# Nilau1998/SAC-Agent

Measured on AMD Instinct MI355X. Metric: env-steps/sec (whole node), boat_env exp-6, 65 536 envs/GPU at 1/2/4/8 MI355X, higher is better.
Workload: dtype f64

## Files before the change

sac-agent_amd/csrc/sacenv_boat.hip:

```cpp

#include <hip/hip_runtime.h>
#include <stdint.h>

#include "sacenv.h"
#include "sacenv_boat_arena.h"
#include "sacenv_boat_math.h"
#include "sacenv_boat_wind.h"
#include "sacenv_boat_draw.h"
#include "sacenv_toys.h"
#include "sacenv_boat_owner.h"

#pragma clang fp contract(off)

namespace {


__global__ void k_spline_g(SacenvBoatParams p, double* __restrict__ g) {
  if (threadIdx.x != 0 || blockIdx.x != 0) return;
  const int n = p.n_knots;
  double a[kMaxK][kMaxK], r[kMaxK][kMaxK];
  for (int i = 0; i < n; ++i)
    for (int j = 0; j < n; ++j) a[i][j] = r[i][j] = 0.0;
  a[0][0] = 1.0, a[0][1] = -2.0, a[0][2] = 1.0;
  a[n - 1][n - 3] = 1.0, a[n - 1][n - 2] = -2.0, a[n - 1][n - 1] = 1.0;
  for (int j = 1; j < n - 1; ++j) {
    a[j][j - 1] = 1.0, a[j][j] = 4.0, a[j][j + 1] = 1.0;
    r[j][j - 1] = 1.0, r[j][j] = -2.0, r[j][j + 1] = 1.0;
  }
  for (int c = 0; c < n; ++c) {
    int piv = c;
    for (int i = c + 1; i < n; ++i)
      if (fabs(a[i][c]) > fabs(a[piv][c])) piv = i;
    for (int j = 0; j < n; ++j) {
      double t = a[c][j]; a[c][j] = a[piv][j]; a[piv][j] = t;
      t = r[c][j]; r[c][j] = r[piv][j]; r[piv][j] = t;
    }
    const double d = a[c][c];
    for (int j = 0; j < n; ++j) a[c][j] /= d, r[c][j] /= d;
    for (int i = 0; i < n; ++i) {
      if (i == c) continue;
      const double f = a[i][c];
      if (f == 0.0) continue;
      for (int j = 0; j < n; ++j) a[i][j] -= f * a[c][j], r[i][j] -= f * r[c][j];
    }
  }
  for (int i = 0; i < n; ++i)
    for (int j = 0; j < n; ++j) g[i * n + j] = r[i][j];
}

constexpr int kMaskThreads = 1024;

__global__ void __launch_bounds__(kWave) k_seed(SacenvBoatParams p, Arena A, const uint32_t* __restrict__ seeds) {
  const int e = blockIdx.x * kWave + threadIdx.x;
  if (e < A.nwaves()) A.refill_mask()[e] = 0ull;
  if (e >= p.n_envs) return;
  uint32_t x = seeds[e];
  uint32_t* key = A.mt_key() + (int64_t)e * kMtN;
  for (int i = 0; i < kMtN; ++i) {
    key[i] = x;
    x = 1812433253u * (x ^ (x >> 30)) + (uint32_t)(i + 1);
  }
  A.i32(U_MTPOS)[e] = kMtN;
  A.i32(U_CONS)[e] = 0;
  A.i32(U_FILL)[e] = 0;
}

__global__ void __launch_bounds__(kWave) k_draw(SacenvBoatParams p, Arena A, Tail T, int mode,
                                                const int32_t* __restrict__ ids,
                                                const int32_t* __restrict__ ex_start_y,
                                                const double* __restrict__ ex_knots,
                                                const int32_t* __restrict__ dev_count) {
  __shared__ DrawLds lds;
  const int lane = threadIdx.x;
  const int nq = dev_count != nullptr ? *dev_count : (int)gridDim.x;
  if ((int)blockIdx.x >= nq) return;
  load_g(p, T.g, lds, lane);
  for (int q = blockIdx.x; q < nq; q += gridDim.x) {
    const int e = ids != nullptr ? ids[q] : q;
    if (e < 0 || e >= p.n_envs) continue;
    int32_t start_y;
    int slot = 0;
    if (mode == 2) {
      start_y = draw_episode_wave(p, A, lds, e, 0, lane, ex_start_y + q,
                                  ex_knots != nullptr ? ex_knots + (int64_t)q * 2 * p.n_knots : nullptr);
    } else if (!p.autoreset) {
      start_y = draw_episode_wave(p, A, lds, e, 0, lane, nullptr, nullptr);
    } else if (mode == 0) {
      start_y = draw_episode_wave(p, A, lds, e, 0, lane, nullptr, nullptr);
      if (lane == 0) {
        A.i32(U_CONS)[e] = 0;
        A.i32(U_FILL)[e] = 1;
      }
    } else {
      const int c = A.i32(U_CONS)[e] + 1;
      const int f = A.i32(U_FILL)[e];
      if (c >= f && lane == 0) atomicOr(&A.status()[1], SACENV_STATUS_SLOT_UNDERFLOW);
      slot = c % kSlots;
      start_y = A.i32(U_STARTY)[(int64_t)slot * A.np + e];
      if (lane == 0) A.i32(U_CONS)[e] = c;
      draw_episode_wave(p, A, lds, e, f % kSlots, lane, nullptr, nullptr);
      if (lane == 0) A.i32(U_FILL)[e] = f + 1;
    }
    if (lane == 0) {
      const Obs o = fresh_state(p, A, T, e, start_y, slot);
      store_obs(A.obs() + (int64_t)e * SACENV_OBS_DIM, o);
    }
    __syncthreads();
  }
}

__global__ void __launch_bounds__(1024) k_compact(const uint8_t* __restrict__ done, int n, int aligned,
                                                  int32_t* __restrict__ ids, int32_t* __restrict__ count) {
  __shared__ int wsum[16];
  __shared__ int base_s;
  const int t = threadIdx.x, lane = t & 63, w = t >> 6;
  if (t == 0) base_s = 0;
  __syncthreads();
  for (int64_t c0 = 0; c0 < n; c0 += 1024 * 64) {
    const int64_t e0 = c0 + (int64_t)t * 64;
    uint64_t bits = 0;
    if (aligned && e0 + 64 <= n) {
      const uint4* v = reinterpret_cast<const uint4*>(done + e0);
#pragma unroll
      for (int k = 0; k < 4; ++k) {
        const uint4 x = v[k];
        const uint32_t wds[4] = {x.x, x.y, x.z, x.w};
#pragma unroll
        for (int d = 0; d < 4; ++d)
#pragma unroll
          for (int by = 0; by < 4; ++by)
            if ((wds[d] >> (8 * by)) & 0xffu) bits |= 1ull << (16 * k + 4 * d + by);
      }
    } else {
      for (int j = 0; j < 64 && e0 + j < n; ++j)
        if (done[e0 + j]) bits |= 1ull << j;
    }
    const int cnt = __popcll(bits);
    const int incl = wave_incl_scan(cnt);
    if (lane == 63) wsum[w] = incl;
    __syncthreads();
    int wbase = 0;
    for (int k = 0; k < w; ++k) wbase += wsum[k];
    int pos = base_s + wbase + incl - cnt;
    while (bits) {
      const int j = __ffsll((long long)bits) - 1;
      bits &= bits - 1ull;
      ids[pos++] = (int32_t)(e0 + j);
    }
    __syncthreads();
    if (t == 1023) base_s += wbase + incl;
    __syncthreads();
  }
  if (t == 0) *count = base_s;
}

#ifdef SACENV_STAMPS
#define REFILL_STAMP(slot, ...)                                     \
  do {                                                              \
    asm volatile("" ::__VA_ARGS__);                                 \
    (slot) = __builtin_amdgcn_s_memrealtime();                      \
  } while (0)
constexpr int kRefillStamps = 24;
#else
#define REFILL_STAMP(slot, ...) \
  do {                          \
  } while (0)
#endif

constexpr int kGroupLanes = 16;
constexpr int kGroups = kWave / kGroupLanes;
__global__ void __launch_bounds__(kWave) k_refill(SacenvBoatParams p, Arena A) {
  __shared__ RngLds lds;
  const int lane = threadIdx.x;
#ifdef SACENV_STAMPS
  uint64_t stm[kRefillStamps] = {};
  int n_st = 0;
#endif
  REFILL_STAMP(stm[0], "s"(lane));
  const int total = __builtin_amdgcn_readfirstlane(A.status()[2]);
  REFILL_STAMP(stm[1], "s"(total));
  if (blockIdx.x == 0 && lane == 0) A.status()[0] += 1;
  const int G = (int)gridDim.x;
  const int g = lane / kGroupLanes, gl = lane % kGroupLanes;
  const int nk = p.n_knots;
  const int ndraw = n_curves(p.experiment);
  const int ncurves = owner_curves(p);
  const int need = 2 * nk * ndraw;
  const int nwords = kGroupLanes + need;
  const bool grp_ok = nk <= 8;
  const uint32_t rng = (uint32_t)(2 * p.start_y_half - 1), mask = range_mask32(rng);
  const int np_ = (int)A.np;
  int r0 = blockIdx.x * kGroups;
  int rq = r0 + g < np_ ? r0 + g : 0;
  int e_n = A.refill_list(0)[rq], f_n = A.refill_list(1)[rq], c_n = A.refill_list(2)[rq], p_n = A.cons_snap()[rq];
  for (; r0 < total; r0 += kGroups * G) {
    const int rr = r0 + g;
    const bool ok = rr < total;
    const int e = ok ? e_n : 0;
    const int c = ok ? c_n : 0;
    const int f0 = ok ? f_n : 0;
    const int pos = ok ? (p_n & kMtPosMask) : kMtN;
    const bool nx = ok && (p_n & kMtNextOk) != 0;
    if (r0 + kGroups * G < total) {
      rq = rr + kGroups * G < np_ ? rr + kGroups * G : 0;
      e_n = A.refill_list(0)[rq], f_n = A.refill_list(1)[rq], c_n = A.refill_list(2)[rq], p_n = A.cons_snap()[rq];
    }
    if (ok && c >= f0 && gl == 0) atomicOr(&A.status()[1], SACENV_STATUS_SLOT_UNDERFLOW);
    const int f_end = ok && f0 < c + kSlots ? c + kSlots : f0;
    int f_next = f0, pos_next = pos;
    bool live = ok && f0 < f_end && grp_ok;
    uint32_t* const gw = lds.blk[0] + g * 3 * kGroupLanes;
#pragma unroll 1
    while (__ballot(live) != 0ull) {
      bool fast = live && pos_next + nwords <= (nx ? 2 * kMtN : kMtN);
      const int64_t eo = (int64_t)e * kMtN;
      uint32_t w[3];
#pragma unroll
      for (int q = 0; q < 3; ++q) {
        const int i = pos_next + gl + kGroupLanes * q;
        const uint32_t* src = i < kMtN ? A.mt_key() + eo + i : A.mt_next() + eo + (i - kMtN);
        w[q] = fast && gl + kGroupLanes * q < nwords ? mt_temper(*src) : 0u;
      }
      wave_lds_sync();
#pragma unroll
      for (int q = 0; q < 3; ++q) gw[gl + kGroupLanes * q] = w[q];
      const unsigned long long acc = __ballot(fast && (w[0] & mask) <= rng);
      const uint32_t gacc = (uint32_t)(acc >> (kGroupLanes * g)) & 0xFFFFu;
      fast = fast && gacc != 0u;
      const int k = fast ? __builtin_ctz(gacc) : 0;
      wave_lds_sync();
      REFILL_STAMP(stm[2], "v"(k));
      if (fast) {
        const int slot = f_next % kSlots;
        const int cc = gl / 8, jj = gl % 8;
        if (cc < ncurves && jj < nk) {
          const int src = k + 1 + cc * 2 * nk + 2 * jj;
          const double kv = res53(gw[src], gw[src + 1]);
          A.wind_knots()[2 * A.wix(slot, cc, jj, e)] = kv;
          if (A.rk) A.knots_raw()[A.wix(slot, cc, jj, e)] = kv;
        }
        if (gl == 0) {
          A.i32(U_STARTY)[(int64_t)slot * A.np + e] = -p.start_y_half + (int32_t)(gw[k] & mask);
          A.i32(U_MTPOS)[e] = (pos_next + k + 1 + need) | (nx ? kMtNextOk : 0);
        }
        f_next = f_next + 1;
        pos_next = pos_next + k + 1 + need;
      }
      live = fast && f_next < f_end;
    }
    wave_lds_sync();
#pragma unroll 1
    for (int j = 0; j < kGroups; ++j) {
      const int src = j * kGroupLanes;
      if (__builtin_amdgcn_readlane((int)ok, src) == 0) break;
      const int ej = __builtin_amdgcn_readlane(e, src);
      const int fe = __builtin_amdgcn_readlane(f_end, src);
      int f = __builtin_amdgcn_readlane(f_next, src);
      const int pj = __builtin_amdgcn_readlane(pos_next, src);
      bool first = true;
      for (; f < fe; ++f) {
        const int32_t start_y = draw_knots_wave(p, A, lds, ej, lane, nullptr, nullptr, first ? pj : -1);
#ifdef SACENV_STAMPS
        const int sb = 3 + (n_st < 18 ? n_st : 18);
        ++n_st;
#endif
        REFILL_STAMP(stm[sb], "v"(start_y));
        first = false;
        __syncthreads();
        store_draw(p, A, lds, ej, f % kSlots, start_y, lane, true);
        __syncthreads();
      }
      if (lane == 0) {
        A.i32(U_FILL)[ej] = fe;
        A.refill_list(1)[r0 + j] = __builtin_amdgcn_readlane(f0, src);
        A.refill_list(2)[r0 + j] = fe;
      }
    }
  }
#ifdef SACENV_STAMPS
  stm[22] = __builtin_amdgcn_s_memrealtime();
  stm[23] = (uint64_t)n_st;
  if (lane == 0 && (int64_t)(blockIdx.x + 1) * kRefillStamps * 8 <= 24 * A.np) {
    uint64_t* d = reinterpret_cast<uint64_t*>(A.accel()) + (int64_t)blockIdx.x * kRefillStamps;
    for (int i = 0; i < kRefillStamps; ++i) d[i] = stm[i];
  }
#endif
}

template <int GS, bool kFull>
__global__ void __launch_bounds__(kWave) k_refill_fit(SacenvBoatParams p, Arena A, Tail T) {
  const int lane = threadIdx.x;
  const int ahead = (int)(A.np / kAheadEnvs);
  if ((int)blockIdx.x < ahead) {
    mt_ahead(p, A, (int)blockIdx.x, lane);
    return;
  }
  const int fb = (int)blockIdx.x - ahead, fgrid = (int)gridDim.x - ahead;
  const int nc = p.use_wind_table ? 0 : n_curves(p.experiment);
  const int nk = kFull ? GS : p.n_knots;
  const int items = A.status()[2] * nc;
#ifdef SACENV_STAMPS
  const uint64_t st0 = __builtin_amdgcn_s_memrealtime();
  uint64_t* const fst = reinterpret_cast<uint64_t*>(A.reward64()) + 2 * (int64_t)blockIdx.x;
  const bool fst_ok = lane == 0 && (int64_t)(blockIdx.x + 1) * 16 <= 8 * A.np;
  if (fst_ok) fst[0] = st0, fst[1] = 0;
#endif
  if (items == 0 || fb * (kWave / GS) >= items) return;
  const int j = lane & (GS - 1);
  const int jj = j < nk ? j : nk - 1, j1 = jj + 1 < nk ? jj + 1 : jj;
  double gr[GS];
#pragma unroll
  for (int k = 0; k < GS; ++k) gr[k] = kFull || k < nk ? T.g[jj * nk + k] : 0.0;
  IvGrid ig = interval_grid(p, j < nk - 1 ? j : 0);
  ig.valid = ig.valid && j < nk - 1;
  const int per = kWave / GS;
  for (int base = fb * per; base < items; base += fgrid * per) {
    const int item = base + lane / GS;
    if (item >= items) break;
    fit_group<GS, kFull>(p, A, gr, ig, item, j, jj, j1, nc);
  }
#ifdef SACENV_STAMPS
  __syncthreads();
  if (fst_ok) fst[1] = __builtin_amdgcn_s_memrealtime();
#endif
}

__device__ __forceinline__ unsigned long long lookback_load(const unsigned long long* w) {
  return __hip_atomic_load(w, __ATOMIC_RELAXED, __HIP_MEMORY_SCOPE_AGENT);
}
__global__ void __launch_bounds__(kMaskThreads) k_need_masks(SacenvBoatParams p, Arena A) {
  __shared__ int wcnt[kMaskThreads / kWave];
  const int t = threadIdx.x, lane = t & (kWave - 1), wv = t >> 6;
  const int nw = A.nwaves(), b = (int)blockIdx.x;
  const int w = b * (kMaskThreads / kWave) + wv, e = w * kWave + lane;
  const uint32_t epoch = (uint32_t)A.status()[0] + 1u;
  bool need = false;
  int c = 0, fl = 0, mp = 0;
  if (w < nw && e < p.n_envs) {
    c = A.i32(U_CONS)[e];
    fl = A.i32(U_FILL)[e];
    mp = A.i32(U_MTPOS)[e];
    need = fl < c + kSlots;
  }
  const unsigned long long m = __ballot(need);
  if (lane == 0) wcnt[wv] = __popcll(m);
  __syncthreads();
  if (t < kWave) {
    unsigned long long* const look = A.refill_mask();
    const int cnt = t < kMaskThreads / kWave ? wcnt[t] : 0;
    const int incl = wave_incl_scan(cnt);
    const int total = __builtin_amdgcn_readlane(incl, kMaskThreads / kWave - 1);
    if (t == 0)
      __hip_atomic_store(look + b, ((unsigned long long)epoch << 32) | (uint32_t)total, __ATOMIC_RELAXED,
                         __HIP_MEMORY_SCOPE_AGENT);
    int before = 0;
    for (int q0 = 0; q0 < b; q0 += kWave) {
      const int q = q0 + t;
      unsigned long long x = q < b ? lookback_load(look + q) : ((unsigned long long)epoch << 32);
      for (uint32_t it = 0; __ballot((uint32_t)(x >> 32) != epoch) != 0ull; ++it) {
        if (it >= kSpinLimit) {
          if (t == 0) atomicOr(&A.status()[1], SACENV_STATUS_LIST_TIMEOUT);
          break;
        }
        __builtin_amdgcn_s_sleep(1);
        if ((uint32_t)(x >> 32) != epoch) x = lookback_load(look + q);
      }
      int v = (uint32_t)(x >> 32) == epoch ? (int)(uint32_t)x : 0;
      v += __shfl_xor(v, 32);
      v += __shfl_xor(v, 16);
      v += __shfl_xor(v, 8);
      v += __shfl_xor(v, 4);
      v += __shfl_xor(v, 2);
      v += __shfl_xor(v, 1);
      before += v;
    }
    if (t < kMaskThreads / kWave) wcnt[t] = before + incl - cnt;
    if (t == 0 && b == (int)gridDim.x - 1) A.status()[2] = before + total;
  }
  __syncthreads();
  if (need) {
    const int r = wcnt[wv] + __popcll(m & ((1ull << lane) - 1ull));
    A.refill_list(0)[r] = e;
    A.refill_list(1)[r] = fl;
    A.refill_list(2)[r] = c;
    A.cons_snap()[r] = mp;
  }
}

template <bool kMixed, int kNc, bool kTIdx>
__global__ void __launch_bounds__(kWave) k_step(SacenvBoatParams p, Arena A, Tail T,
                                                const float* __restrict__ action, int nb_boat,
                                                MixedToys M, char* __restrict__ trans) {
  __shared__ OwnerLds slds;
  const int lane = threadIdx.x;
  int b = (int)blockIdx.x;
  if (!kMixed || b < nb_boat) {
    owner_wave<false, kNc, kTIdx>(p, A, T, action, slds, b, lane, 1, nullptr,
                                  trans);
    return;
  }
  b -= nb_boat;
  if (b < M.nb[0]) {
    toy_wave(M.p[0], M.a[0], b, lane);
  } else if (M.n > 1) {
    toy_wave(M.p[1], M.a[1], b - M.nb[0], lane);
  }
}

template <int kNc, bool kTIdx, int kRows, bool kLean = false>
__global__ void __launch_bounds__(kWave) k_rollout(SacenvBoatParams p, Arena A, Tail T,
                                                   const float* __restrict__ action, int n_steps, RollArgs ra) {
  __shared__ OwnerLds slds;
  rollout_body<kNc, kTIdx, kRows, true, kLean>(p, A, T, action, n_steps, ra, slds);
}
template <int kNc, bool kTIdx, int kRows, bool kLean = false>
__global__ void __launch_bounds__(kWave) __attribute__((amdgpu_waves_per_eu(2, 2)))
k_rollout_dense(SacenvBoatParams p, Arena A, Tail T, const float* __restrict__ action, int n_steps, RollArgs ra) {
  __shared__ OwnerLds slds;
  rollout_body<kNc, kTIdx, kRows, false, kLean>(p, A, T, action, n_steps, ra, slds);
}

template <int kNc, bool kTIdx, bool kLean = false>
__global__ void __launch_bounds__(kWave) k_rollout_mixed(SacenvBoatParams p, Arena A, Tail T,
                                                         const float* __restrict__ action, int n_steps, RollArgs ra,
                                                         int nb_boat, MixedToys M) {
  __shared__ OwnerLds slds;
  const int lane = threadIdx.x;
  int b = (int)blockIdx.x;
  if (b < nb_boat) {
    owner_wave<true, kNc, kTIdx, false, 0, true, kLean>(vreg_params(p), A, vreg_tail(T), action, slds, b, lane,
                                                         n_steps, &ra);
    return;
  }
  b -= nb_boat;
  if (b < M.nb[0]) {
    toy_roll_wave(M.p[0], M.a[0], b, lane, n_steps);
  } else if (M.n > 1) {
    toy_roll_wave(M.p[1], M.a[1], b - M.nb[0], lane, n_steps);
  }
}

__global__ void __launch_bounds__(kWave) k_toy_init(SacenvToyParams p, ToyArena T, const int32_t* __restrict__ ids,
                                                    int n, int zero_counters) {
  const int q = blockIdx.x * kWave + threadIdx.x;
  if (q >= n) return;
  const int e = ids != nullptr ? ids[q] : q;
  if (e < 0 || e >= p.n_envs) return;
  double f[5];
  float obs[2];
  toy_initial(p, f, obs);
  for (int k = 0; k < 5; ++k) T.f(k)[e] = f[k];
  T.count()[e] = 0;
  if (zero_counters)
    for (int k = 0; k < 3; ++k) T.ctr(k)[e] = 0u;
  reinterpret_cast<float2*>(T.obs())[e] = make_float2(obs[0], obs[1]);
  T.reward()[e] = 0.0f;
  T.done()[e] = 0;
  T.term()[e] = 0;
}

__global__ void __launch_bounds__(kWave) k_toy_step(SacenvToyParams p, ToyArena T) {
  toy_wave(p, T, blockIdx.x, threadIdx.x);
}

__global__ void __launch_bounds__(256) k_wind_eval(SacenvBoatParams p, Arena A, Tail T,
                                                   const int32_t* __restrict__ env_ids,
                                                   const int32_t* __restrict__ idx, int n,
                                                   double* __restrict__ out_v, double* __restrict__ out_a) {
  const int q = blockIdx.x * blockDim.x + threadIdx.x;
  if (q >= n) return;
  const int e = env_ids[q];
  if (e < 0 || e >= p.n_envs) return;
  const int slot = p.autoreset ? A.i32(U_CONS)[e] % kSlots : 0;
  double wv, wa;
  wind_at(p, A, T.table, slot, e, idx[q], wv, wa);
  out_v[q] = wv;
  out_a[q] = wa;
}


int check_params(const SacenvBoatParams* p) {
  if (p == nullptr) return SACENV_E_NULL;
  if (p->experiment < 1 || p->experiment > 6) return SACENV_E_EXPERIMENT;
  if (p->n_envs <= 0 || p->n_envs > (1 << 22) || p->wind_len <= 0) return SACENV_E_SIZE;
  if (n_curves(p->experiment) > 0 && (p->n_knots < 4 || p->n_knots > kMaxK)) return SACENV_E_KNOTS;
  if (p->n_knots < 2 || p->n_knots > kMaxK) return SACENV_E_KNOTS;
  if (n_curves(p->experiment) > 0 && !p->use_wind_table && p->wind_len < 2) return SACENV_E_SIZE;
  if (p->start_y_half < 1) return SACENV_E_RANGE;
  if (p->autoreset && (p->n_helpers < 1 || p->n_helpers > 65536)) return SACENV_E_SIZE;
  return SACENV_OK;
}

Tail make_tail(const SacenvBoatParams& p, void* arena) {
  const Arena A = make_arena(p, arena);
  Tail T;
  T.g = reinterpret_cast<const double*>(A.b + off_spline_g(A.ur(), A.np));
  T.table = reinterpret_cast<const double*>(A.b + off_wind_table(A.ur(), A.np));
  T.r_mx = 1.0 / p.m_plus_mx;
  T.r_my = 1.0 / p.m_plus_my;
  T.r_iz = 1.0 / p.i_plus_iz;
  T.r_nd = 1.0 / p.n_times_d;
  T.r_w = 1.0 / p.track_width;
  T.r_goal = 1.0 / p.goal_line;
  T.r_two_w = 1.0 / (p.track_width + p.track_width);
  T.r_fuel = 1.0 / (double)p.fuel0;
  T.k_front = p.c_r_front * 0.5 * p.rho * p.boat_area_front;
  T.k_thrust = p.n_squared * p.rho * p.d_pow4 * p.one_minus_td;
  T.k_side = p.c_r_side * 0.5 * p.rho * p.boat_area_side;
  T.k_rud_front = p.c_r_front * 0.5 * p.rho * p.rudder_area;
  T.k_hull = p.c_r_side * 0.5 * p.rho * p.boat_area_side * p.boat_l * 5.0;
  T.k_rud_moment = p.c_r_side * 0.5 * p.rho * p.rudder_area * (p.boat_b / 2);
  return T;
}

int launch_status() {
  const hipError_t err = hipGetLastError();
  return err == hipSuccess ? SACENV_OK : (int)err;
}

inline int blocks_for(int n, int per) { return (n + per - 1) / per; }
inline int owner_waves(const SacenvBoatParams& p) { return (int)(pad64(p.n_envs) / kWave); }

int check_toy(const SacenvToyParams* p) {
  if (p == nullptr) return SACENV_E_NULL;
  if (p->kind != SACENV_TOY_PARACHUTE && p->kind != SACENV_TOY_CAR) return SACENV_E_EXPERIMENT;
  if (p->n_envs <= 0) return SACENV_E_SIZE;
  return SACENV_OK;
}

ToyArena make_toy_arena(const SacenvToyParams& p, void* base) {
  return ToyArena{static_cast<char*>(base), pad64(p.n_envs)};
}

using StepKernel = void (*)(SacenvBoatParams, Arena, Tail, const float*, int, MixedToys, char*);
using RolloutKernel = void (*)(SacenvBoatParams, Arena, Tail, const float*, int, RollArgs);
using MixedRolloutKernel = void (*)(SacenvBoatParams, Arena, Tail, const float*, int, RollArgs, int, MixedToys);
using FitKernel = void (*)(SacenvBoatParams, Arena, Tail);

template <int kNc, bool kTIdx>
struct Owner {
  static constexpr int nc = kNc;
  static constexpr bool ti = kTIdx;
};
template <class F>
auto owner_dispatch(const SacenvBoatParams& p, F f) {
  switch (owner_curves(p) * 2 + (t_from_index(p.dt) ? 1 : 0)) {
    case 0: return f(Owner<0, false>{});
    case 1: return f(Owner<0, true>{});
    case 2: return f(Owner<1, false>{});
    case 3: return f(Owner<1, true>{});
    case 4: return f(Owner<2, false>{});
    default: return f(Owner<2, true>{});
  }
}

StepKernel step_kernel(const SacenvBoatParams& p, bool mixed) {
  return owner_dispatch(p, [mixed](auto o) -> StepKernel {
    using O = decltype(o);
    return mixed ? k_step<true, O::nc, O::ti> : k_step<false, O::nc, O::ti>;
  });
}

bool dense_grid(int nb_boat) {
  int dev = 0, cus = 0;
  if (hipGetDevice(&dev) != hipSuccess ||
      hipDeviceGetAttribute(&cus, hipDeviceAttributeMultiprocessorCount, dev) != hipSuccess)
    return false;
  return nb_boat > 4 * cus;
}

bool lean_launch(const SacenvBoatParams& p, const RollArgs& ra) {
  return p.out_flags == 0 && p.autoreset != 0 && p.experiment != 2 && p.fuel0 != 0 && ra.rec_stride == 0 &&
         ra.fin_stride == 0;
}

int rollout_rows(const RollArgs& ra) {
  return ra.stage != nullptr ? 2 : ra.trans != nullptr ? 1 : ra.rec_stride != 0 ? 3 : 0;
}

template <int kNc, bool kTIdx, int kRows, bool kLean = false>
RolloutKernel rollout_one(bool dense) {
  return dense ? k_rollout_dense<kNc, kTIdx, kRows, kLean> : k_rollout<kNc, kTIdx, kRows, kLean>;
}
RolloutKernel rollout_kernel(const SacenvBoatParams& p, int rows, bool lean, bool dense) {
  return owner_dispatch(p, [=](auto o) -> RolloutKernel {
    constexpr int nc = decltype(o)::nc;
    constexpr bool ti = decltype(o)::ti;
    switch (rows) {
      case 0: return lean ? rollout_one<nc, ti, 0, true>(dense) : rollout_one<nc, ti, 0>(dense);
      case 1: return rollout_one<nc, ti, 1>(dense);
      case 2: return lean ? rollout_one<nc, ti, 2, true>(dense) : rollout_one<nc, ti, 2>(dense);
      default: return rollout_one<nc, ti, 3>(dense);
    }
  });
}

MixedRolloutKernel rollout_mixed_kernel(const SacenvBoatParams& p, bool lean) {
  return owner_dispatch(p, [lean](auto o) -> MixedRolloutKernel {
    using O = decltype(o);
    return lean ? k_rollout_mixed<O::nc, O::ti, true> : k_rollout_mixed<O::nc, O::ti>;
  });
}

FitKernel refill_fit_kernel(int n_knots) {
  return n_knots == 8   ? k_refill_fit<8, true>
         : n_knots < 8  ? k_refill_fit<8, false>
         : n_knots == 16 ? k_refill_fit<16, true>
                         : k_refill_fit<16, false>;
}

RollArgs arena_roll_args(const Arena& A) {
  RollArgs ra{};
  ra.rec = A.b + A.ur() * A.np;
  ra.fin = reinterpret_cast<float*>(ra.rec + R_FIN * A.np);
  ra.status = reinterpret_cast<int32_t*>(A.b + off_status(A.ur(), A.np)) + 1;
  return ra;
}

int launch_multi(const SacenvBoatParams& p, void* arena, const float* actions, int n_steps, const RollArgs& ra,
                 void* stream) {
  const int nb_boat = owner_waves(p);
  const RolloutKernel k = rollout_kernel(p, rollout_rows(ra), lean_launch(p, ra), dense_grid(nb_boat));
  hipLaunchKernelGGL(k, dim3(nb_boat), dim3(kWave), 0, (hipStream_t)stream, p, make_arena(p, arena),
                     make_tail(p, arena), actions, n_steps, ra);
  return launch_status();
}

struct MixedLaunch {
  MixedToys M{};
  SacenvBoatParams p{};
  Arena A{};
  Tail T{};
  int nb_boat = 0, nb = 0;
};
int mixed_setup(const SacenvBoatParams* bp, void* boat_arena, const float* boat_actions,
                const SacenvToyParams* toy_params, void* const* toy_arenas, int32_t n_toys, int32_t n_steps,
                MixedLaunch* L) {
  int rc;
  if (n_toys < 0 || n_toys > 2) return SACENV_E_SIZE;
  if (n_toys > 0 && (toy_params == nullptr || toy_arenas == nullptr)) return SACENV_E_NULL;
  if (n_steps < 1) return SACENV_E_SIZE;
  L->M.n = n_toys;
  for (int t = 0; t < n_toys; ++t) {
    if ((rc = check_toy(&toy_params[t]))) return rc;
    if (toy_arenas[t] == nullptr) return SACENV_E_NULL;
    L->M.p[t] = toy_params[t];
    L->M.a[t] = make_toy_arena(toy_params[t], toy_arenas[t]);
    L->M.nb[t] = blocks_for(toy_params[t].n_envs, kWave);
    L->nb += L->M.nb[t];
  }
  if (bp != nullptr) {
    if ((rc = check_params(bp))) return rc;
    if (boat_arena == nullptr || boat_actions == nullptr) return SACENV_E_NULL;
    L->p = *bp;
    L->A = make_arena(*bp, boat_arena);
    L->T = make_tail(*bp, boat_arena);
    L->nb_boat = owner_waves(*bp);
    L->nb += L->nb_boat;
  }
  return SACENV_OK;
}

}

extern "C" {

int sacenv_abi_version(void) { return SACENV_ABI_VERSION; }

int sacenv_stream_create_exclusive(void** stream) {
  if (stream == nullptr) return SACENV_E_NULL;
  int dev = 0;
  hipError_t e = hipGetDevice(&dev);
  if (e != hipSuccess) return (int)e;
  hipDeviceProp_t prop;
  e = hipGetDeviceProperties(&prop, dev);
  if (e != hipSuccess) return (int)e;
  uint32_t mask[64];
  const int words = (prop.multiProcessorCount + 31) / 32;
  if (words > 64) return SACENV_E_SIZE;
  for (int i = 0; i < words; ++i) mask[i] = 0xFFFFFFFFu;
  hipStream_t s = nullptr;
  e = hipExtStreamCreateWithCUMask(&s, (uint32_t)words, mask);
  if (e != hipSuccess) return (int)e;
  *stream = s;
  return SACENV_OK;
}

int sacenv_stream_destroy(void* stream) {
  if (stream == nullptr) return SACENV_E_NULL;
  return (int)hipStreamDestroy((hipStream_t)stream);
}

const char* sacenv_error_string(int code) {
  switch (code) {
    case SACENV_OK: return "ok";
    case SACENV_E_NULL: return "required pointer is NULL";
    case SACENV_E_EXPERIMENT: return "Well someone tried to use an experiment that doesnt exist!";
    case SACENV_E_KNOTS:
      return "Please select at least 4 fixed_points in your config. The interpolation doesn't work "
             "otherwise! (max 16)";
    case SACENV_E_SIZE: return "size out of range";
    case SACENV_E_RANGE: return "low >= high: int(0.8*track_width) must be >= 1";
    case SACENV_E_MODE: return "call not valid in this autoreset mode";
    default: return code > 0 ? hipGetErrorString((hipError_t)code) : "unknown sacenv error";
  }
}

int sacenv_boat_layout(const SacenvBoatParams* p, SacenvBoatLayout* out) {
  const int rc = check_params(p);
  if (rc) return rc;
  if (out == nullptr) return SACENV_E_NULL;
  compute_layout(p->n_envs, p->n_knots, p->wind_len, p->use_wind_table, (p->out_flags & SACENV_OUT_KNOTS) != 0, out);
  return SACENV_OK;
}

int sacenv_boat_init(const SacenvBoatParams* p, void* arena, const uint32_t* seeds, void* stream) {
  int rc = check_params(p);
  if (rc) return rc;
  if (arena == nullptr || seeds == nullptr) return SACENV_E_NULL;
  const hipStream_t s = (hipStream_t)stream;
  const Arena A = make_arena(*p, arena);
  const Tail T = make_tail(*p, arena);
  hipLaunchKernelGGL(k_spline_g, dim3(1), dim3(1), 0, s, *p, const_cast<double*>(T.g));
  if ((rc = launch_status())) return rc;
  hipLaunchKernelGGL(k_seed, dim3(blocks_for(p->n_envs, kWave)), dim3(kWave), 0, s, *p, A, seeds);
  if ((rc = launch_status())) return rc;
  hipLaunchKernelGGL(k_draw, dim3(p->n_envs), dim3(kWave), 0, s, *p, A, T, 0, (const int32_t*)nullptr,
                     (const int32_t*)nullptr, (const double*)nullptr, (const int32_t*)nullptr);
  if ((rc = launch_status())) return rc;
  return p->autoreset ? sacenv_boat_refill(p, arena, stream) : SACENV_OK;
}

int sacenv_boat_reset(const SacenvBoatParams* p, void* arena, const int32_t* ids, int32_t n_ids,
                      void* stream) {
  int rc = check_params(p);
  if (rc) return rc;
  if (arena == nullptr) return SACENV_E_NULL;
  const int nb = ids != nullptr ? n_ids : p->n_envs;
  if (nb < 0) return SACENV_E_SIZE;
  if (nb == 0) return SACENV_OK;
  const hipStream_t s = (hipStream_t)stream;
  const Arena A = make_arena(*p, arena);
  const Tail T = make_tail(*p, arena);
  hipLaunchKernelGGL(k_draw, dim3(nb), dim3(kWave), 0, s, *p, A, T, 1, ids, (const int32_t*)nullptr,
                     (const double*)nullptr, (const int32_t*)nullptr);
  return launch_status();
}

int sacenv_compact_done(const uint8_t* done, int32_t n, int32_t* ids, int32_t* count, void* stream) {
  if (n < 0) return SACENV_E_SIZE;
  if (count == nullptr || (n > 0 && (done == nullptr || ids == nullptr))) return SACENV_E_NULL;
  const int aligned = (reinterpret_cast<uintptr_t>(done) & 15u) == 0;
  hipLaunchKernelGGL(k_compact, dim3(1), dim3(1024), 0, (hipStream_t)stream, done, n, aligned, ids, count);
  return launch_status();
}

int sacenv_boat_reset_list(const SacenvBoatParams* p, void* arena, const int32_t* ids, const int32_t* count,
                           void* stream) {
  int rc = check_params(p);
  if (rc) return rc;
  if (arena == nullptr || ids == nullptr || count == nullptr) return SACENV_E_NULL;
  const hipStream_t s = (hipStream_t)stream;
  const Arena A = make_arena(*p, arena);
  const Tail T = make_tail(*p, arena);
  const int grid = p->n_envs < 1024 ? p->n_envs : 1024;
  hipLaunchKernelGGL(k_draw, dim3(grid), dim3(kWave), 0, s, *p, A, T, 1, ids, (const int32_t*)nullptr,
                     (const double*)nullptr, count);
  return launch_status();
}

int sacenv_boat_reset_explicit(const SacenvBoatParams* p, void* arena, const int32_t* ids, int32_t n_ids,
                               const int32_t* start_y, const double* knots, void* stream) {
  int rc = check_params(p);
  if (rc) return rc;
  if (p->autoreset) return SACENV_E_MODE;
  if (arena == nullptr || ids == nullptr || start_y == nullptr) return SACENV_E_NULL;
  if (n_curves(p->experiment) > 0 && !p->use_wind_table && knots == nullptr) return SACENV_E_NULL;
  if (n_ids < 0) return SACENV_E_SIZE;
  if (n_ids == 0) return SACENV_OK;
  hipLaunchKernelGGL(k_draw, dim3(n_ids), dim3(kWave), 0, (hipStream_t)stream, *p, make_arena(*p, arena),
                     make_tail(*p, arena), 2, ids, start_y, knots, (const int32_t*)nullptr);
  return launch_status();
}

static int boat_step(const SacenvBoatParams* p, void* arena, const float* action, char* trans, void* stream) {
  int rc = check_params(p);
  if (rc) return rc;
  if (arena == nullptr || action == nullptr) return SACENV_E_NULL;
  const int nb_boat = owner_waves(*p);
  hipLaunchKernelGGL(step_kernel(*p, false), dim3(nb_boat), dim3(kWave), 0, (hipStream_t)stream, *p,
                     make_arena(*p, arena), make_tail(*p, arena), action, nb_boat, MixedToys{}, trans);
  return launch_status();
}

int sacenv_boat_step(const SacenvBoatParams* p, void* arena, const float* action, void* stream) {
  return boat_step(p, arena, action, nullptr, stream);
}

int sacenv_boat_step_pooled(const SacenvBoatParams* p, void* arena, const float* action, void* trans,
                            void* stream) {
  if (trans == nullptr) return SACENV_E_NULL;
  if ((reinterpret_cast<uintptr_t>(trans) & 15u) != 0u) return SACENV_E_RANGE;
  return boat_step(p, arena, action, static_cast<char*>(trans), stream);
}

int sacenv_boat_rollout(const SacenvBoatParams* p, void* arena, const float* actions, int32_t n_steps,
                        void* records, float* final_obs, void* stream) {
  int rc = check_params(p);
  if (rc) return rc;
  if (arena == nullptr || actions == nullptr || records == nullptr) return SACENV_E_NULL;
  if (n_steps < 1 || (p->autoreset && n_steps > SACENV_REFILL_PERIOD)) return SACENV_E_SIZE;
  const int64_t np = pad64(p->n_envs);
  RollArgs ra{};
  ra.rec = static_cast<char*>(records);
  ra.rec_stride = SACENV_RECORD_BYTES * np;
  ra.fin = final_obs;
  ra.fin_stride = np * SACENV_OBS_DIM;
  ra.act_stride = p->n_envs;
  return launch_multi(*p, arena, actions, n_steps, ra, stream);
}

int sacenv_boat_segment(const SacenvBoatParams* p, void* arena, const float* actions, int64_t action_stride,
                        int32_t n_steps, const uint32_t* act_ready, uint32_t* step_done, uint32_t seq0,
                        void* trans, int64_t trans_stride, void* stage, uint64_t* stage_marks,
                        void* stream) {
  int rc = check_params(p);
  if (rc) return rc;
  if (arena == nullptr || actions == nullptr) return SACENV_E_NULL;
  if (n_steps < 1 || (p->autoreset && n_steps > SACENV_REFILL_PERIOD)) return SACENV_E_SIZE;
  if (action_stride < p->n_envs ||
      ((act_ready != nullptr || step_done != nullptr) && (uint64_t)seq0 + (uint64_t)n_steps >= 0x80000000ull))
    return SACENV_E_RANGE;
  if (trans != nullptr && ((reinterpret_cast<uintptr_t>(trans) & 15u) != 0u || (trans_stride & 15) != 0))
    return SACENV_E_RANGE;
  if (stage != nullptr && (trans != nullptr || (reinterpret_cast<uintptr_t>(stage) & 15u) != 0u))
    return SACENV_E_RANGE;
  if (stage_marks != nullptr && n_steps > SACENV_REFILL_PERIOD) return SACENV_E_SIZE;
  RollArgs ra = arena_roll_args(make_arena(*p, arena));
  ra.trans = static_cast<char*>(trans);
  ra.trans_stride = trans_stride;
  ra.stage = static_cast<char*>(stage);
  ra.marks = reinterpret_cast<unsigned long long*>(stage_marks);
  ra.act_stride = action_stride;
  ra.ready = act_ready;
  ra.done = step_done;
  ra.seq0 = seq0;
  return launch_multi(*p, arena, actions, n_steps, ra, stream);
}

int sacenv_boat_segment_occupancy(const SacenvBoatParams* p, int32_t with_trans, int32_t* blocks_per_cu,
                                  int32_t* grid, int32_t* vgprs, int32_t* lds_bytes) {
  int rc = check_params(p);
  if (rc) return rc;
  if (blocks_per_cu == nullptr || grid == nullptr || vgprs == nullptr || lds_bytes == nullptr) return SACENV_E_NULL;
  const int nb_boat = owner_waves(*p);
  const int rows = with_trans == 2 ? 2 : with_trans ? 1 : 0;
  const RolloutKernel k = rollout_kernel(*p, rows, lean_launch(*p, RollArgs{}), dense_grid(nb_boat));
  int nb = 0;
  hipFuncAttributes fa{};
  hipError_t e = hipOccupancyMaxActiveBlocksPerMultiprocessor(&nb, k, kWave, 0);
  if (e == hipSuccess) e = hipFuncGetAttributes(&fa, reinterpret_cast<const void*>(k));
  if (e != hipSuccess) return (int)e;
  *blocks_per_cu = nb;
  *grid = nb_boat;
  *vgprs = fa.numRegs;
  *lds_bytes = (int32_t)fa.sharedSizeBytes;
  return SACENV_OK;
}

int sacenv_boat_refill(const SacenvBoatParams* p, void* arena, void* stream) {
  int rc = check_params(p);
  if (rc) return rc;
  if (arena == nullptr) return SACENV_E_NULL;
  if (!p->autoreset) return SACENV_E_MODE;
  const Arena A = make_arena(*p, arena);
  const unsigned mask_blocks = (unsigned)((A.np / kWave + kMaskThreads / kWave - 1) / (kMaskThreads / kWave));
  hipLaunchKernelGGL(k_need_masks, dim3(mask_blocks), dim3(kMaskThreads), 0, (hipStream_t)stream, *p, A);
  if ((rc = launch_status())) return rc;
  hipLaunchKernelGGL(k_refill, dim3(p->n_helpers), dim3(kWave), 0, (hipStream_t)stream, *p, A);
  if ((rc = launch_status())) return rc;
  const int fit_blocks = 8192 + (int)(A.np / kAheadEnvs);
  hipLaunchKernelGGL(refill_fit_kernel(p->n_knots), dim3(fit_blocks), dim3(kWave), 0, (hipStream_t)stream, *p, A,
                     make_tail(*p, arena));
  return launch_status();
}

int sacenv_toy_layout(const SacenvToyParams* p, SacenvToyLayout* out) {
  const int rc = check_toy(p);
  if (rc) return rc;
  if (out == nullptr) return SACENV_E_NULL;
  toy_layout(p->n_envs, out);
  return SACENV_OK;
}

int sacenv_toy_init(const SacenvToyParams* p, void* arena, void* stream) {
  const int rc = check_toy(p);
  if (rc) return rc;
  if (arena == nullptr) return SACENV_E_NULL;
  hipLaunchKernelGGL(k_toy_init, dim3(blocks_for(p->n_envs, kWave)), dim3(kWave), 0, (hipStream_t)stream, *p,
                     make_toy_arena(*p, arena), (const int32_t*)nullptr, p->n_envs, 1);
  return launch_status();
}

int sacenv_toy_reset(const SacenvToyParams* p, void* arena, const int32_t* ids, int32_t n_ids, void* stream) {
  const int rc = check_toy(p);
  if (rc) return rc;
  if (arena == nullptr) return SACENV_E_NULL;
  const int n = ids != nullptr ? n_ids : p->n_envs;
  if (n < 0) return SACENV_E_SIZE;
  if (n == 0) return SACENV_OK;
  hipLaunchKernelGGL(k_toy_init, dim3(blocks_for(n, kWave)), dim3(kWave), 0, (hipStream_t)stream, *p,
                     make_toy_arena(*p, arena), ids, n, 0);
  return launch_status();
}

int sacenv_toy_step(const SacenvToyParams* p, void* arena, void* stream) {
  const int rc = check_toy(p);
  if (rc) return rc;
  if (arena == nullptr) return SACENV_E_NULL;
  hipLaunchKernelGGL(k_toy_step, dim3(blocks_for(p->n_envs, kWave)), dim3(kWave), 0, (hipStream_t)stream, *p,
                     make_toy_arena(*p, arena));
  return launch_status();
}

static int mixed_step(const SacenvBoatParams* bp, void* boat_arena, const float* boat_action,
                      const SacenvToyParams* toy_params, void* const* toy_arenas, int32_t n_toys,
                      char* trans, void* stream) {
  MixedLaunch L;
  const int rc = mixed_setup(bp, boat_arena, boat_action, toy_params, toy_arenas, n_toys, 1, &L);
  if (rc) return rc;
  if (L.nb == 0) return SACENV_OK;
  hipLaunchKernelGGL(step_kernel(L.p, true), dim3(L.nb), dim3(kWave), 0, (hipStream_t)stream, L.p, L.A, L.T,
                     boat_action, L.nb_boat, L.M, trans);
  return launch_status();
}

int sacenv_mixed_step(const SacenvBoatParams* bp, void* boat_arena, const float* boat_action,
                      const SacenvToyParams* toy_params, void* const* toy_arenas, int32_t n_toys,
                      void* stream) {
  return mixed_step(bp, boat_arena, boat_action, toy_params, toy_arenas, n_toys, nullptr, stream);
}

int sacenv_mixed_step_pooled(const SacenvBoatParams* bp, void* boat_arena, const float* boat_action,
                             const SacenvToyParams* toy_params, void* const* toy_arenas, int32_t n_toys,
                             void* trans, void* stream) {
  if (bp == nullptr || trans == nullptr) return SACENV_E_NULL;
  if ((reinterpret_cast<uintptr_t>(trans) & 15u) != 0u) return SACENV_E_RANGE;
  return mixed_step(bp, boat_arena, boat_action, toy_params, toy_arenas, n_toys, static_cast<char*>(trans),
                    stream);
}

int sacenv_mixed_segment(const SacenvBoatParams* bp, void* boat_arena, const float* boat_actions,
                         int64_t action_stride, int32_t n_steps, const SacenvToyParams* toy_params,
                         void* const* toy_arenas, int32_t n_toys, void* stream) {
  MixedLaunch L;
  const int rc = mixed_setup(bp, boat_arena, boat_actions, toy_params, toy_arenas, n_toys, n_steps, &L);
  if (rc) return rc;
  RollArgs ra{};
  if (bp != nullptr) {
    if (bp->autoreset && n_steps > SACENV_REFILL_PERIOD) return SACENV_E_SIZE;
    if (action_stride < bp->n_envs) return SACENV_E_RANGE;
    ra = arena_roll_args(L.A);
    ra.act_stride = action_stride;
  }
  if (L.nb == 0) return SACENV_OK;
  hipLaunchKernelGGL(rollout_mixed_kernel(L.p, lean_launch(L.p, ra)), dim3(L.nb), dim3(kWave), 0,
                     (hipStream_t)stream, L.p, L.A, L.T, boat_actions, n_steps, ra, L.nb_boat, L.M);
  return launch_status();
}

int sacenv_boat_wind_eval(const SacenvBoatParams* p, const void* arena, const int32_t* env_ids,
                          const int32_t* idx, int32_t n, double* out_velocity, double* out_angle,
                          void* stream) {
  int rc = check_params(p);
  if (rc) return rc;
  if (!arena || !env_ids || !idx || !out_velocity || !out_angle) return SACENV_E_NULL;
  if (n < 0) return SACENV_E_SIZE;
  if (n == 0) return SACENV_OK;
  void* a = const_cast<void*>(arena);
  hipLaunchKernelGGL(k_wind_eval, dim3(blocks_for(n, 256)), dim3(256), 0, (hipStream_t)stream, *p,
                     make_arena(*p, a), make_tail(*p, a), env_ids, idx, n, out_velocity, out_angle);
  return launch_status();
}

}
```

sac-agent_amd/csrc/sacenv_boat_arena.h:

```cpp
#pragma once

#include <hip/hip_runtime.h>
#include <stdint.h>
#include <string.h>

#include "sacenv.h"

namespace {
constexpr int kWave = 64;
}

#include "mt19937.h"

namespace {

constexpr int kMaxK = SACENV_MAX_KNOTS;
constexpr int kSlots = SACENV_SLOTS;
constexpr double kPi = 3.141592653589793;

constexpr int U_SX = 0, U_SY = 8, U_SR = 16, U_VX = 24, U_VY = 32, U_VR = 40, U_RUD = 48,
              U_EP = 56, U_COEF = 64, U_W0N = 128, U_T = 144, U_IDX = 152,
              U_CONS = 156, U_FILL = 160, U_MTPOS = 164, U_SYN = 168, U_STARTY = 172,
              U_CNT = U_STARTY + 4 * kSlots,
              U_LIST = U_CNT + 4 * SACENV_N_COUNTERS, U_CSNAP = U_LIST + 12, U_LTERM = U_CSNAP + 4,
              U_WIND = U_LTERM + 4;
constexpr int U_MT_BYTES = 4 * kMtN;
constexpr int kMtPosMask = 0xFFFF, kMtNextOk = 1 << 16;
constexpr int U_PAIRED = 144;
constexpr int64_t kWindUnits = 16LL * kSlots;

__host__ __device__ inline int64_t pad64(int64_t n) { return (n + 63) / 64 * 64; }
__host__ __device__ inline int64_t align256(int64_t x) { return (x + 255) / 256 * 256; }

constexpr int R_OBS = SACENV_REC_OBS, R_REWARD = SACENV_REC_REWARD, R_DONE = SACENV_REC_DONE,
              R_TERM = SACENV_REC_TERM, R_FIN = SACENV_RECORD_BYTES,
              R_FIN_EP = R_FIN + 4 * SACENV_OBS_DIM,
              R_AX = R_FIN_EP + 8, R_AY = R_AX + 8, R_AR = R_AY + 8,
              R_REWARD64 = R_AR + 8, R_END = R_REWARD64 + 8;
static_assert(R_OBS == 0 && R_REWARD == 4 * SACENV_OBS_DIM && R_DONE == R_REWARD + 4 && R_TERM == R_DONE + 1 &&
                  SACENV_RECORD_BYTES == R_TERM + 1,
              "record: obs f32 x 11, reward f32, done u8, term u8");
static_assert(R_FIN == 50 && R_FIN_EP == 94 && R_AX == 102 && R_AY == 110 && R_AR == 118 && R_REWARD64 == 126 &&
                  R_END == 134,
              "the arena columns behind the record (SacenvBoatLayout, ABI 20)");
static_assert(R_FIN_EP % 2 == 0 && (R_AX - R_FIN_EP) % 8 == 0, "f64 columns stay 8-B aligned (n_pad % 64 == 0)");

__host__ __device__ inline int64_t record_unit(int nk, int rk) {
  return U_WIND + (2 + rk) * (kWindUnits * nk) + 2 * U_MT_BYTES;
}
__host__ __device__ inline int64_t off_refill_mask(int64_t ur, int64_t np) { return align256((ur + R_END) * np); }
__host__ __device__ inline int64_t refill_mask_bytes(int64_t np) { return align256(8 * (int)(np / 64)); }
__host__ __device__ inline int64_t off_status(int64_t ur, int64_t np) {
  return off_refill_mask(ur, np) + refill_mask_bytes(np);
}
__host__ __device__ inline int64_t off_spline_g(int64_t ur, int64_t np) { return off_status(ur, np) + 256; }
__host__ __device__ inline int64_t off_wind_table(int64_t ur, int64_t np) {
  return off_spline_g(ur, np) + align256(8LL * kMaxK * kMaxK);
}

__host__ __device__ inline void compute_layout(int n, int nk, int L, int use_table, int raw_knots,
                                               SacenvBoatLayout* o) {
  const int64_t np = pad64(n);
  o->n_pad = np;
  auto pair_off = [np](int u) { return (int64_t)(u & ~15) * np + (u & 8); };
  o->s_x = pair_off(U_SX);
  o->s_y = pair_off(U_SY);
  o->s_r = pair_off(U_SR);
  o->v_x = pair_off(U_VX);
  o->v_y = pair_off(U_VY);
  o->v_r = pair_off(U_VR);
  o->rudder = pair_off(U_RUD);
  o->t = U_T * np;
  o->ep_reward = pair_off(U_EP);
  o->wind_coef = U_COEF * np;
  o->wind0_next = U_W0N * np;
  o->start_y_next = U_SYN * np;
  o->index = U_IDX * np;
  o->cons = U_CONS * np;
  o->fill = U_FILL * np;
  o->mt_pos = U_MTPOS * np;
  o->start_y = U_STARTY * np;
  o->counters = U_CNT * np;
  o->refill_list = U_LIST * np;
  const int64_t uw = U_WIND, wk = kWindUnits * nk, rk = raw_knots ? 1 : 0;
  o->wind_knots = uw * np;
  o->knots_raw = raw_knots ? (uw + 2 * wk) * np : -1;
  o->mt_key = (uw + (2 + rk) * wk) * np;
  o->mt_next = o->mt_key + U_MT_BYTES * np;
  const int64_t ur = record_unit(nk, (int)rk);
  o->record = ur * np;
  o->obs = (ur + R_OBS) * np;
  o->reward = (ur + R_REWARD) * np;
  o->done = (ur + R_DONE) * np;
  o->term = (ur + R_TERM) * np;
  o->final_obs = (ur + R_FIN) * np;
  o->final_ep_reward = (ur + R_FIN_EP) * np;
  o->accel = (ur + R_AX) * np;
  o->reward64 = (ur + R_REWARD64) * np;
  o->refill_mask = off_refill_mask(ur, np);
  o->status = off_status(ur, np);
  o->spline_g = off_spline_g(ur, np);
  o->wind_table = off_wind_table(ur, np);
  o->total_bytes = o->wind_table + (use_table ? align256(16LL * L) : 0);
  o->last_term = U_LTERM * np;
}

struct Arena {
  char* b;
  int64_t np;
  int nk;
  int rk;
  template <class T>
  __device__ __forceinline__ T* at(int64_t units) const { return reinterpret_cast<T*>(b + units * np); }
  __device__ __forceinline__ int32_t* i32(int u) const { return at<int32_t>(u); }
  __device__ __forceinline__ int nwaves() const { return (int)(np / 64); }
  __device__ __forceinline__ int64_t wk() const { return kWindUnits * nk; }
  __device__ __forceinline__ double* wind_knots() const { return at<double>(U_WIND); }
  __device__ __forceinline__ double* knots_raw() const { return at<double>(U_WIND + 2 * wk()); }
  __device__ __forceinline__ uint32_t* mt_key() const { return at<uint32_t>(U_WIND + (2 + rk) * wk()); }
  __device__ __forceinline__ uint32_t* mt_next() const { return mt_key() + kMtN * np; }
  __host__ __device__ __forceinline__ int64_t ur() const { return record_unit(nk, rk); }
  __device__ __forceinline__ float* obs() const { return at<float>(ur() + R_OBS); }
  __device__ __forceinline__ float* final_obs() const { return at<float>(ur() + R_FIN); }
  __device__ __forceinline__ double* accel() const { return at<double>(ur() + R_AX); }
  __device__ __forceinline__ double* reward64() const { return at<double>(ur() + R_REWARD64); }
  __device__ __forceinline__ char* tail() const { return b + off_refill_mask(ur(), np); }
  __device__ __forceinline__ unsigned long long* refill_mask() const {
    return reinterpret_cast<unsigned long long*>(tail());
  }

  __device__ __forceinline__ int32_t* cons_snap() const { return i32(U_CSNAP); }
  __device__ __forceinline__ int32_t* status() const {
    return reinterpret_cast<int32_t*>(tail() + refill_mask_bytes(np));
  }
  __device__ __forceinline__ int32_t* refill_list(int k) const { return i32(U_LIST + 4 * k); }
  __device__ __forceinline__ int64_t wix(int slot, int c, int k, int e) const {
    return (((int64_t)e * kSlots + slot) * 2 + c) * nk + k;
  }
  __device__ __forceinline__ const char* wk_wave(int e0) const {
    return reinterpret_cast<const char*>(wind_knots()) + (int64_t)e0 * (int64_t)kSlots * 32 * nk;
  }
  __device__ __forceinline__ uint32_t wko_l(int slot, int c, int k, int l) const {
    return ((((uint32_t)l * (uint32_t)kSlots + (uint32_t)slot) * 2u + (uint32_t)c) * (uint32_t)nk + (uint32_t)k) * 16u;
  }
  __device__ __forceinline__ void piece_at(const char* wbase, uint32_t off, double (&q)[4]) const {
    const char* base = wbase + off;
    const double2 a = *reinterpret_cast<const double2*>(base), b = *reinterpret_cast<const double2*>(base + 16);
    q[0] = a.x, q[1] = a.y, q[2] = b.x, q[3] = b.y;
  }
  __device__ __forceinline__ void piece(int slot, int c, int k, int e, double (&q)[4]) const {
    piece_at(wk_wave(e & ~63), wko_l(slot, c, k, e & 63), q);
  }
  template <class T>
  __device__ __forceinline__ T& at_e(int64_t unit, uint32_t off) const {
    return *reinterpret_cast<T*>(b + unit * np + off);
  }
  template <class T>
  __device__ __forceinline__ T& at_s(int u, uint32_t off) const {
    return *reinterpret_cast<T*>(b + ((uint32_t)u * (uint32_t)np + off));
  }
  __device__ __forceinline__ double& f64e(int u, uint32_t eo) const {
    return u < U_PAIRED ? at_s<double>(u & ~15, 2u * eo + (uint32_t)(u & 8)) : at_s<double>(u, eo);
  }
  __device__ __forceinline__ double2& f64p(int u, uint32_t eo) const { return at_s<double2>(u, 2u * eo); }
  __device__ __forceinline__ int32_t& i32e(int u, uint32_t eo4) const { return at_s<int32_t>(u, eo4); }
};

__host__ inline Arena make_arena(const SacenvBoatParams& p, void* base) {
  return Arena{static_cast<char*>(base), pad64(p.n_envs), p.n_knots, (p.out_flags & SACENV_OUT_KNOTS) ? 1 : 0};
}

struct Tail {
  const double* g;
  const double* table;
  double r_mx, r_my, r_iz, r_nd, r_w;
  double r_goal, r_two_w, r_fuel;
  double k_front, k_thrust, k_side, k_rud_front, k_hull, k_rud_moment;
};

__host__ __device__ __forceinline__ int n_curves(int experiment) {
  return experiment == 6 ? 2 : (experiment == 4 || experiment == 5) ? 1 : 0;
}
__host__ __device__ __forceinline__ int owner_curves(const SacenvBoatParams& p) {
  return p.use_wind_table ? 0 : n_curves(p.experiment);
}

__host__ __device__ inline bool t_from_index(double dt) {
  uint64_t bits;
  memcpy(&bits, &dt, sizeof bits);
  return (bits & ((1ull << 30) - 1ull)) == 0ull;
}

}
```

sac-agent_amd/csrc/sacenv_boat_draw.h:

```cpp
#pragma once

#include <hip/hip_runtime.h>
#include <stdint.h>

#include "sacenv.h"
#include "sacenv_boat_arena.h"
#include "sacenv_boat_math.h"
#include "sacenv_boat_wind.h"
#include "mt19937.h"

#pragma clang fp contract(off)

namespace {

struct RngLds {
  uint32_t win[kWave];
  uint32_t blk[2][kMtN];
  double y[2][kMaxK];
};
struct DrawLds : RngLds {
  double m[2][kMaxK];
  double g[kMaxK * kMaxK];
};


__device__ __forceinline__ void load_g(const SacenvBoatParams& p, const double* g, DrawLds& l, int lane) {
  for (int i = lane; i < p.n_knots * p.n_knots; i += kWave) l.g[i] = g[i];
  __syncthreads();
}


__device__ int32_t draw_knots_wave(const SacenvBoatParams& p, const Arena& A, RngLds& l, int e,
                                   int lane, const int32_t* ex_start_y, const double* ex_knots,
                                   int pos0 = -1, bool have_w0 = false, uint32_t w0_pre = 0u) {
  const int nk = p.n_knots;
  const int ndraw = n_curves(p.experiment);
  const int ncurves = owner_curves(p);
  if (ex_start_y != nullptr) {
    for (int c = 0; c < ncurves; ++c)
      if (lane < nk) l.y[c][lane] = ex_knots[c * nk + lane];
    return *ex_start_y;
  }
  MtStream st;
  st.gkey = A.mt_key() + (int64_t)e * kMtN;
  st.pos = pos0 >= 0 ? pos0 : A.i32(U_MTPOS)[e] & kMtPosMask;
  st.cur = 0;
  st.loaded = false;
  st.nxt_valid = false;
  st.advanced = false;
  const uint32_t rng = (uint32_t)(2 * p.start_y_half - 1), mask = range_mask32(rng);
  uint32_t val = 0;
  const int need = 2 * nk * ndraw;
  const uint32_t w0 = have_w0 ? mt_temper(w0_pre) : mt_fetch(st, l, lane);
  const unsigned long long acc0 = __ballot(((w0 & mask) <= rng) && lane < kWave - need);
  if (acc0) {
    const int k = __ffsll((long long)acc0) - 1;
    val = (uint32_t)__builtin_amdgcn_readlane((int)w0, k) & mask;
    if (ndraw > 0) {
      l.win[lane] = w0;
      __syncthreads();
    }
    for (int c = 0; c < ndraw; ++c) {
      const int src = k + 1 + c * 2 * nk + ((2 * lane) & 31);
      const uint32_t wa = l.win[src & (kWave - 1)];
      const uint32_t wb = l.win[(src + 1) & (kWave - 1)];
      if (lane < nk) l.y[c][lane] = res53(wa, wb);
    }
    st.pos += k + 1 + need;
  } else {
    for (;;) {
      const uint32_t w = mt_fetch(st, l, lane);
      const unsigned long long acc = __ballot((w & mask) <= rng);
      if (acc) {
        const int k = __ffsll((long long)acc) - 1;
        val = (uint32_t)__builtin_amdgcn_readlane((int)w, k) & mask;
        st.pos += k + 1;
        break;
      }
      st.pos += kWave;
    }
    for (int c = 0; c < ndraw; ++c) {
      const uint32_t w = mt_fetch(st, l, lane);
      l.win[lane] = w;
      __syncthreads();
      const uint32_t wa = l.win[(2 * lane) & (kWave - 1)];
      const uint32_t wb = l.win[(2 * lane + 1) & (kWave - 1)];
      if (lane < nk) l.y[c][lane] = res53(wa, wb);
      __syncthreads();
      st.pos += 2 * nk;
    }
  }
  mt_finish(st, l, A.i32(U_MTPOS) + e, lane);
  return -p.start_y_half + (int32_t)val;
}

__device__ void fit_store_wave(const SacenvBoatParams& p, const Arena& A, DrawLds& l, int e, int slot,
                               int lane) {
  const int nk = p.n_knots;
  const int ncurves = owner_curves(p);
  if (ncurves == 0) return;
  __syncthreads();
  const int c = lane >> 4, j = lane & 15;
  const bool knot_lane = c < ncurves && j < nk;
  double yv = 0.0, mv = 0.0;
  if (knot_lane) {
    yv = l.y[c][j];
#pragma unroll
    for (int k = 0; k < kMaxK; ++k)
      if (k < nk) mv += l.g[j * nk + k] * l.y[c][k];
    l.m[c][j] = mv;
  }
  __syncthreads();
  double mn = INFINITY, mx = -INFINITY;
  {
    const int cc = lane >> 5, u = lane & 31;
    if (nk - 1 <= 8) {
      const int jj = u >> 2;
      if (cc < ncurves && jj < nk - 1)
        interval_extrema<4>(p, jj, u & 3, l.y[cc][jj], l.y[cc][jj + 1], l.m[cc][jj], l.m[cc][jj + 1], mn, mx);
    } else {
      if (cc < ncurves && u < nk - 1)
        interval_extrema<1>(p, u, 0, l.y[cc][u], l.y[cc][u + 1], l.m[cc][u], l.m[cc][u + 1], mn, mx);
    }
  }
  mn = group_min<16>(mn);
  mx = group_max<16>(mx);
  const double cmn0 = fmin(readlane_f64(mn, 0), readlane_f64(mn, 16));
  const double cmx0 = fmax(readlane_f64(mx, 0), readlane_f64(mx, 16));
  const double cmn1 = fmin(readlane_f64(mn, 32), readlane_f64(mn, 48));
  const double cmx1 = fmax(readlane_f64(mx, 32), readlane_f64(mx, 48));
  mn = c == 0 ? cmn0 : cmn1;
  mx = c == 0 ? cmx0 : cmx1;
  if (knot_lane) {
    fold_knot(p, c, mn, mx, yv, mv);
    *reinterpret_cast<double2*>(A.wind_knots() + 2 * A.wix(slot, c, j, e)) = double2{yv, mv};
  }
  __syncthreads();
}

__device__ __forceinline__ void store_draw(const SacenvBoatParams& p, const Arena& A, const RngLds& l,
                                           int e, int slot, int32_t start_y, int lane, bool raw = false) {
  const int nk = p.n_knots;
  const int ncurves = owner_curves(p);
  if (lane == 0) A.i32(U_STARTY)[(int64_t)slot * A.np + e] = start_y;
  const int c = lane >> 4, j = lane & 15;
  if (c < ncurves && j < nk) {
    if (raw) A.wind_knots()[2 * A.wix(slot, c, j, e)] = l.y[c][j];
    if (A.rk) A.knots_raw()[A.wix(slot, c, j, e)] = l.y[c][j];
  }
}

__device__ int32_t draw_episode_wave(const SacenvBoatParams& p, const Arena& A, DrawLds& l, int e,
                                     int slot, int lane, const int32_t* ex_start_y,
                                     const double* ex_knots) {
  const int32_t start_y = draw_knots_wave(p, A, l, e, lane, ex_start_y, ex_knots);
  __syncthreads();
  store_draw(p, A, l, e, slot, start_y, lane);
  fit_store_wave(p, A, l, e, slot, lane);
  return start_y;
}

__device__ __forceinline__ Obs fresh_state(const SacenvBoatParams& p, const Arena& A, const Tail& T, int e,
                                           int32_t start_y, int slot) {
  const double s_y = p.experiment == 2 ? (double)start_y : 0.0;
  const int nc = owner_curves(p);
  const uint32_t eo = (uint32_t)e * 8u;
  for (int c = 0; c < nc; ++c) {
    double q[4];
    A.piece(slot, c, 0, e, q);
    for (int k = 0; k < 4; ++k) A.f64e(U_COEF + 32 * c + 8 * k, eo) = q[k];
  }
  A.f64e(U_SX, eo) = 0.0;
  A.f64e(U_SY, eo) = s_y;
  A.f64e(U_SR, eo) = 0.0;
  A.f64e(U_VX, eo) = 0.0;
  A.f64e(U_VY, eo) = 0.0;
  A.f64e(U_VR, eo) = 0.0;
  A.f64e(U_RUD, eo) = 0.0;
  A.f64e(U_T, eo) = 0.0;
  A.f64e(U_EP, eo) = 0.0;
  A.i32(U_IDX)[e] = 0;
  if (p.out_flags & SACENV_OUT_ACCEL) {
    A.at_e<double>(A.ur() + R_AX, eo) = 0.0;
    A.at_e<double>(A.ur() + R_AY, eo) = 0.0;
    A.at_e<double>(A.ur() + R_AR, eo) = 0.0;
  }
  return make_obs(p, obs_const(T), 0.0, 0.0, 0.0, s_y, 0.0, 0.0, 0.0, 0.0, 0.0, 0.0, (double)p.fuel0);
}

constexpr int kAheadEnvs = 8;
__device__ __forceinline__ void mt_twist_regs(const uint32_t* o, uint32_t* n, uint32_t* cur, int lane) {
  constexpr int kD = kMtN - kMtM;
  uint32_t a0[4], a1[4], a2[4], b0[4], b1[4], c0[4], c1[4];
#pragma unroll
  for (int k = 0; k < 4; ++k) {
    const int c = lane + kWave * k;
    const bool ok = c < kD, okc = c < kMtN - 1 - 2 * kD;
    a0[k] = ok ? o[c] : 0u;
    a1[k] = ok ? o[c + 1] : 0u;
    a2[k] = ok ? o[c + kMtM] : 0u;
    b0[k] = ok ? o[c + kD] : 0u;
    b1[k] = ok ? o[c + kD + 1] : 0u;
    c0[k] = okc ? o[c + 2 * kD] : 0u;
    c1[k] = okc ? o[c + 2 * kD + 1] : 0u;
  }
  const uint32_t last = o[kMtN - 1];
  asm volatile("s_waitcnt vmcnt(0)" ::: "memory");
  uint32_t nb2 = 0u, na0 = 0u;
#pragma unroll
  for (int k = 0; k < 4; ++k) {
    const int c = lane + kWave * k;
    if (c < kD) {
      const uint32_t na = mt_mix(a0[k], a1[k], a2[k]);
      const uint32_t nb = mt_mix(b0[k], b1[k], na);
      n[c] = na;
      n[c + kD] = nb;
      if (cur) cur[c] = a0[k], cur[c + kD] = b0[k];
      if (c < kMtN - 1 - 2 * kD) {
        n[c + 2 * kD] = mt_mix(c0[k], c1[k], nb);
        if (cur) cur[c + 2 * kD] = c0[k];
      }
      if (k == 0) na0 = na;
      if (k == 2) nb2 = nb;
    }
  }
  const uint32_t n0 = (uint32_t)__builtin_amdgcn_readlane((int)na0, 0);
  const uint32_t n396 = (uint32_t)__builtin_amdgcn_readlane((int)nb2, kMtM - 1 - kD - 2 * kWave);
  if (lane == 0) {
    n[kMtN - 1] = mt_mix(last, n0, n396);
    if (cur) cur[kMtN - 1] = last;
  }
}

__device__ __forceinline__ void mt_ahead(const SacenvBoatParams& p, const Arena& A, int b, int lane) {
  const int e0 = b * kAheadEnvs;
  int v = 0;
  bool need = false;
  if (lane < kAheadEnvs && e0 + lane < p.n_envs && p.n_knots <= 8) {
    v = A.i32(U_MTPOS)[e0 + lane];
    need = (v & kMtNextOk) == 0 || (v & kMtPosMask) > kMtN;
  }
  unsigned long long m = __ballot(need);
#pragma unroll 1
  while (m != 0ull) {
    const int j = __ffsll((long long)m) - 1;
    m &= m - 1ull;
    const int e = e0 + j;
    const int vj = __builtin_amdgcn_readlane(v, j);
    const bool adv = (vj & kMtNextOk) != 0 && (vj & kMtPosMask) > kMtN;
    uint32_t* const key = A.mt_key() + (int64_t)e * kMtN;
    uint32_t* const nxt = A.mt_next() + (int64_t)e * kMtN;
    mt_twist_regs(adv ? nxt : key, nxt, adv ? key : nullptr, lane);
    if (lane == 0) A.i32(U_MTPOS)[e] = ((vj & kMtPosMask) - (adv ? kMtN : 0)) | kMtNextOk;
  }
}

}
```

sac-agent_amd/csrc/sacenv_boat_wind.h:

```cpp
#pragma once

#include <hip/hip_runtime.h>
#include <stdint.h>

#include "sacenv.h"
#include "sacenv_boat_arena.h"

#pragma clang fp contract(off)

namespace {

struct Knot {
  int j;
  double t;
};

__device__ __forceinline__ Knot knot_coord(const SacenvBoatParams& p, int i) {
  const double s = (double)i * p.knot_step;
  int j = (int)s;
  if (j > p.n_knots - 2) j = p.n_knots - 2;
  return Knot{j, s - (double)j};
}

__device__ __forceinline__ double spline_piece(double y0, double y1, double m0, double m1, double t) {
  const double u = 1.0 - t;
  return u * y0 + t * y1 + (u * u * u - u) * m0 + (t * t * t - t) * m1;
}

__device__ __forceinline__ double curve_env(const SacenvBoatParams& p, const Arena& A, int slot, int c,
                                            int e, int i) {
  const Knot k = knot_coord(p, i);
  double q[4];
  A.piece(slot, c, k.j, e, q);
  return spline_piece(q[0], q[2], q[1], q[3], k.t);
}

__device__ __forceinline__ void wind_at(const SacenvBoatParams& p, const Arena& A, const double* table,
                                        int slot, int e, int idx, double& wv, double& wa) {
  if (idx > p.wind_len - 1) idx = p.wind_len - 1;
  if (idx < 0) idx = 0;
  if (p.use_wind_table) {
    wv = table[idx];
    wa = table[p.wind_len + idx];
    return;
  }
  switch (p.experiment) {
    case 3:
      wv = p.max_velocity;
      wa = p.wind_dir_rad;
      return;
    case 4:
      wv = curve_env(p, A, slot, 0, e, idx);
      wa = p.wind_dir_rad;
      return;
    case 5: {
      wv = p.max_velocity;
      const double r = curve_env(p, A, slot, 0, e, idx) <= 0.5 / 2 ? 0.0 : 1.0;
      wa = (r * kPi) + kPi / 2;
      return;
    }
    case 6:
      wv = curve_env(p, A, slot, 0, e, idx);
      wa = curve_env(p, A, slot, 1, e, idx);
      return;
    default:
      wv = 0.0;
      wa = 0.0;
      return;
  }
}


template <int kCtrl>
__device__ __forceinline__ double dpp_f64(double v) {
  const int lo = __builtin_amdgcn_mov_dpp(__double2loint(v), kCtrl, 0xF, 0xF, false);
  const int hi = __builtin_amdgcn_mov_dpp(__double2hiint(v), kCtrl, 0xF, 0xF, false);
  return __hiloint2double(hi, lo);
}
template <int GS>
__device__ __forceinline__ double group_min(double v) {
  v = fmin(v, dpp_f64<0xB1>(v));
  v = fmin(v, dpp_f64<0x4E>(v));
  v = fmin(v, dpp_f64<0x141>(v));
  if (GS == 16) v = fmin(v, dpp_f64<0x140>(v));
  return v;
}
template <int GS>
__device__ __forceinline__ double group_max(double v) {
  v = fmax(v, dpp_f64<0xB1>(v));
  v = fmax(v, dpp_f64<0x4E>(v));
  v = fmax(v, dpp_f64<0x141>(v));
  if (GS == 16) v = fmax(v, dpp_f64<0x140>(v));
  return v;
}
__device__ __forceinline__ double next_lane_f64(double v) {
  const int lo = __builtin_amdgcn_update_dpp(__double2loint(v), __double2loint(v), 0x101, 0xF, 0xF, false);
  const int hi = __builtin_amdgcn_update_dpp(__double2hiint(v), __double2hiint(v), 0x101, 0xF, 0xF, false);
  return __hiloint2double(hi, lo);
}
__device__ __forceinline__ double readlane_f64(double v, int src) {
  return __hiloint2double(__builtin_amdgcn_readlane(__double2hiint(v), src),
                          __builtin_amdgcn_readlane(__double2loint(v), src));
}
__device__ __forceinline__ void wave_lds_sync() {
  __builtin_amdgcn_fence(__ATOMIC_RELEASE, "wavefront");
  __builtin_amdgcn_wave_barrier();
  __builtin_amdgcn_fence(__ATOMIC_ACQUIRE, "wavefront");
}
__device__ __forceinline__ int wave_incl_scan(int x) {
  x += __builtin_amdgcn_update_dpp(0, x, 0x111, 0xF, 0xF, true);
  x += __builtin_amdgcn_update_dpp(0, x, 0x112, 0xF, 0xF, true);
  x += __builtin_amdgcn_update_dpp(0, x, 0x114, 0xF, 0xF, true);
  x += __builtin_amdgcn_update_dpp(0, x, 0x118, 0xF, 0xF, true);
  x += __builtin_amdgcn_update_dpp(0, x, 0x142, 0xA, 0xF, false);
  x += __builtin_amdgcn_update_dpp(0, x, 0x143, 0xC, 0xF, false);
  return x;
}


struct IvGrid {
  double jd, lod, hid;
  bool valid;
};
__device__ __forceinline__ IvGrid interval_grid(const SacenvBoatParams& p, int j) {
  const int L = p.wind_len;
  int lo = (int)ceil((double)j * p.knot_inv) - 1;
  if (lo < 0) lo = 0;
  while (lo < L && knot_coord(p, lo).j < j) ++lo;
  int hi = (int)floor((double)(j + 1) * p.knot_inv) + 1;
  if (hi > L - 1) hi = L - 1;
  while (hi >= 0 && knot_coord(p, hi).j > j) --hi;
  return IvGrid{(double)j, (double)lo, (double)hi, lo <= hi};
}

template <int S>
__device__ __forceinline__ void interval_extrema_on(const SacenvBoatParams& p, const IvGrid& gr, int s,
                                                    double y0, double y1, double a, double b, double& mn,
                                                    double& mx) {
  mn = INFINITY;
  mx = -INFINITY;
  if (!gr.valid) return;
  const double inv = p.knot_inv;
  const double qa = 3.0 * (b - a), qb = 6.0 * a, qc = y1 - y0 - 2.0 * a - b;
  const double c1 = qc, c2 = 3.0 * a, c3 = b - a;
  double r0 = -1.0, r1 = -1.0;
  const double scale = fabs(qa) + fabs(qb) + fabs(qc);
  if (fabs(qa) <= 1e-14 * scale) {
    if (qb != 0.0) r0 = -qc * __builtin_amdgcn_rcp(qb);
  } else {
    double sa = qa, sb = qb, sc = qc;
    if (scale < 0x1p-500) {
      const int up = -__builtin_amdgcn_frexp_exp(scale);
      sa = ldexp(qa, up), sb = ldexp(qb, up), sc = ldexp(qc, up);
    }
    const double disc = sb * sb - 4.0 * sa * sc;
    if (disc >= 0.0) {
      const double sq = disc > 0.0 ? disc * __builtin_amdgcn_rsq(disc) : 0.0;
      const double q = -0.5 * (sb + copysign(sq, sb));
      r0 = q * __builtin_amdgcn_rcp(sa);
      if (q != 0.0) r1 = sc * __builtin_amdgcn_rcp(q);
    }
  }
  const bool ok0 = r0 > -0.01 && r0 < 1.01, ok1 = r1 > -0.01 && r1 < 1.01;
  const double jd = gr.jd, lod = gr.lod, hid = gr.hid;
  const double i0 = ok0 ? floor((jd + r0) * inv) : lod;
  const double i1 = ok1 ? floor((jd + r1) * inv) : lod;
#pragma unroll
  for (int t = 0; t < (10 + S - 1) / S; ++t) {
    const int q = s + S * t;
    double i;
    if (q == 0) {
      i = lod;
    } else if (q == 1) {
      i = hid;
    } else {
      const bool first = q < 6;
      const double d = (double)((first ? q - 2 : q - 6) - 1);
      const bool ok = first ? ok0 : ok1;
      i = fmin(fmax((first ? i0 : i1) + d, lod), hid);
      i = ok ? i : lod;
    }
    if (q < 10) {
      const double t = i * p.knot_step - jd;
      const double v = fma(fma(fma(c3, t, c2), t, c1), t, y0);
      mn = fmin(mn, v);
      mx = fmax(mx, v);
    }
  }
}
template <int S>
__device__ __forceinline__ void interval_extrema(const SacenvBoatParams& p, int j, int s, double y0,
                                                 double y1, double a, double b, double& mn,
                                                 double& mx) {
  interval_extrema_on<S>(p, interval_grid(p, j), s, y0, y1, a, b, mn, mx);
}

__device__ __forceinline__ void fold_knot(const SacenvBoatParams& p, int c, double mn, double mx, double& yv,
                                          double& mv) {
  if (mn < 0.0 || mx > 1.0) {
    const double span = mx - mn;
    yv = (yv - mn) / span;
    mv = mv / span;
  }
  if (p.experiment == 4 || (p.experiment == 6 && c == 0)) {
    yv = yv * p.max_velocity;
    mv = mv * p.max_velocity;
  } else if (p.experiment == 6 && c == 1) {
    yv = yv * kPi * 2;
    mv = mv * kPi * 2;
  }
}

template <int GS, bool kFull>
__device__ __forceinline__ void fit_group(const SacenvBoatParams& p, const Arena& A, const double (&gr)[GS],
                                          const IvGrid& ig, int item, int j, int jj, int j1, int nc) {
  const int nk = kFull ? GS : p.n_knots;
  const int rr = item / nc, c = item - rr * nc;
  const int e = A.refill_list(0)[rr], f0 = A.refill_list(1)[rr], f1 = A.refill_list(2)[rr];
  for (int f = f0; f < f1; ++f) {
    const int slot = f % kSlots;
    const double* kr = A.wind_knots() + 2 * A.wix(slot, c, 0, e);
    double yk[GS];
#pragma unroll
    for (int k = 0; k < GS; ++k) yk[k] = kr[2 * (kFull || k < nk ? k : nk - 1)];
    double yv = kr[2 * jj];
    const double y1 = kr[2 * j1];
    double mv = 0.0;
#pragma unroll
    for (int k = 0; k < GS; ++k) {
      const double s = mv + gr[k] * yk[k];
      mv = kFull || k < nk ? s : mv;
    }
    const double m1 = next_lane_f64(mv);
    double mn, mx;
    interval_extrema_on<1>(p, ig, 0, yv, y1, mv, m1, mn, mx);
    mn = group_min<GS>(mn);
    mx = group_max<GS>(mx);
    if (kFull || j < nk) {
      fold_knot(p, c, mn, mx, yv, mv);
      *reinterpret_cast<double2*>(A.wind_knots() + 2 * A.wix(slot, c, j, e)) = double2{yv, mv};
    }
  }
}

}
```

sac-agent_amd/sacenv/vec_env.py:

```python
from __future__ import annotations

import ctypes as C

import numpy as np
import torch

from . import _lib
from .config import BoatConfig, make_params, observation_bounds, t_from_index
from .spaces import Box

RECORD_BYTES = _lib.RECORD_BYTES


class VecBoatEnv:

    def __init__(self, config=None, num_envs: int = 1, *, seed: int = 0, seeds=None,
                 device=None, max_episode_steps: int = 0, autoreset: bool = True,
                 env_id_offset: int = 0, record_knots: bool = False, record_accel: bool = False,
                 record_reward64: bool = False, wind_table=None, n_helpers: int | None = None,
                 auto_refill: bool = True):
        self.lib = _lib.load()
        self.cfg = BoatConfig.from_any(config)
        self.num_envs = N = int(num_envs)
        if N <= 0:
            raise ValueError("num_envs must be positive")
        self.device = _lib.cuda_device(device, "VecBoatEnv")
        self.env_id_offset = int(env_id_offset)
        self.autoreset = bool(autoreset)
        self.auto_refill = bool(auto_refill)
        self._since_refill = 0
        if n_helpers is None:
            n_helpers = max(1024, ((N + 63) // 64 * 64) * 3 // 16)
        flags = ((_lib.OUT_KNOTS if record_knots else 0) | (_lib.OUT_ACCEL if record_accel else 0)
                 | (_lib.OUT_REWARD64 if record_reward64 else 0))
        self.params = make_params(self.cfg, N, max_episode_steps=max_episode_steps,
                                  autoreset=autoreset, n_helpers=n_helpers, out_flags=flags,
                                  use_wind_table=wind_table is not None)
        self._pp = C.byref(self.params)
        self.layout = L = _lib.layout(self.params)
        self.n_pad = NP = int(L.n_pad)
        self.arena = torch.zeros(int(L.total_bytes), dtype=torch.uint8, device=self.device)
        nk = int(self.cfg.fixed_points)

        def view(off, dtype, *shape):
            esz = torch.empty((), dtype=dtype).element_size()
            cnt = int(np.prod(shape))
            return self.arena[off: off + cnt * esz].view(dtype).view(*shape)

        f64, i32 = torch.float64, torch.int32

        def pair_view(off):
            k = (off % 16) // 8
            return view(off - 8 * k, f64, NP, 2)[:N, k]

        for name in ("s_x", "s_y", "s_r", "v_x", "v_y", "v_r", "rudder", "ep_reward"):
            setattr(self, name, pair_view(getattr(L, name)))
        self._t_view = view(L.t, f64, NP)[:N]
        self._t_from_index = t_from_index(float(self.cfg.dt))
        self.index = view(L.index, i32, NP)[:N]
        self.cons = view(L.cons, i32, NP)[:N]
        self.mt_pos = view(L.mt_pos, i32, NP)[:N]
        self.start_y_slots = view(L.start_y, i32, _lib.SLOTS, NP)[:, :N]
        self.counters = view(L.counters, i32, _lib.N_COUNTERS, NP)[:, :N]
        self.last_term = view(L.last_term, i32, NP)[:N]
        self.wind_knots = view(L.wind_knots, f64, NP, _lib.SLOTS, 2, nk, 2)
        self.knots_raw_slots = view(L.knots_raw, f64, NP, _lib.SLOTS, 2, nk) if record_knots else None
        self.mt_key = view(L.mt_key, i32, NP, _lib.MT_N)[:N]
        self.mt_next = view(L.mt_next, i32, NP, _lib.MT_N)[:N]
        self.spline_g = view(L.spline_g, f64, nk, nk)
        self.record = self.arena[L.record: L.record + RECORD_BYTES * NP]
        self.obs = view(L.obs, torch.float32, NP, _lib.OBS_DIM)[:N]
        self.reward = view(L.reward, torch.float32, NP)[:N]
        self.done = view(L.done, torch.uint8, NP)[:N]
        self.term = view(L.term, torch.uint8, NP)[:N]
        self.final_obs = view(L.final_obs, torch.float32, NP, _lib.OBS_DIM)[:N]
        self.final_obs_bytes = self.arena[L.final_obs: L.final_obs + 4 * _lib.OBS_DIM * NP]
        self.final_ep_reward = view(L.final_ep_reward, f64, NP)[:N]
        self.accel = view(L.accel, f64, 3, NP)[:, :N]
        self.reward64 = view(L.reward64, f64, NP)[:N]
        self.status = view(L.status, i32, 64)
        if wind_table is not None:
            wt = torch.as_tensor(np.asarray(wind_table, np.float64).reshape(2, -1))
            if wt.shape[1] != self.cfg.wind_len:
                raise ValueError("wind_table must be [2, int(t_max/dt)]")
            view(L.wind_table, f64, 2, self.cfg.wind_len).copy_(wt)

        self.action_space = Box(low=-1, high=1, dtype=np.float32)
        low, high = observation_bounds()
        self.observation_space = Box(low=low, high=high, dtype=np.float32)

        if seeds is None:
            gid = np.arange(N, dtype=np.uint64) + np.uint64(self.env_id_offset)
            seeds = (np.uint64(seed) + gid) & np.uint64(0xFFFFFFFF)
        seeds = np.asarray(seeds, dtype=np.uint64)
        if seeds.shape != (N,):
            raise ValueError("seeds must have one entry per env")
        if np.any(seeds > 0xFFFFFFFF):
            raise ValueError("Seed must be between 0 and 2**32 - 1")
        self.seeds = seeds
        self._seeds_dev = torch.from_numpy(seeds.astype(np.uint32).view(np.int32)).to(self.device)
        _lib.check(self.lib.sacenv_boat_init(self._pp, self._ptr, self._seeds_dev.data_ptr(),
                                             self.stream))

    @property
    def mt_index(self) -> torch.Tensor:
        return self.mt_pos & 0xFFFF

    @property
    def _ptr(self) -> int:
        return self.arena.data_ptr()

    @property
    def stream(self) -> int:
        return torch.cuda.current_stream(self.device).cuda_stream

    @property
    def t(self) -> torch.Tensor:
        if self._t_from_index:
            return self.index.to(torch.float64) * float(self.cfg.dt)
        return self._t_view

    @property
    def start_y(self) -> torch.Tensor:
        slot = (self.cons % _lib.SLOTS).long() if self.autoreset else torch.zeros_like(self.cons).long()
        return self.start_y_slots.gather(0, slot[None, :])[0]

    @property
    def knots_raw(self) -> torch.Tensor:
        if self.knots_raw_slots is None:
            raise RuntimeError("construct the env with record_knots=True to keep the drawn knots")
        slot = (self.cons % _lib.SLOTS).long() if self.autoreset else torch.zeros_like(self.cons).long()
        k = self.knots_raw_slots[: self.num_envs]
        return k[torch.arange(self.num_envs, device=k.device), slot].permute(1, 2, 0)

    def reset(self, env_ids=None) -> torch.Tensor:
        if env_ids is None:
            _lib.check(self.lib.sacenv_boat_reset(self._pp, self._ptr, None, 0, self.stream))
        else:
            ids = torch.as_tensor(env_ids, dtype=torch.int32, device=self.device).contiguous()
            if ids.numel():
                _lib.check(self.lib.sacenv_boat_reset(self._pp, self._ptr, ids.data_ptr(),
                                                      ids.numel(), self.stream))
                self._keep = ids
        return self.obs

    def compact_done(self, done=None):
        d = self.done if done is None else torch.as_tensor(done, dtype=torch.uint8, device=self.device)
        d = d.contiguous()
        ids = torch.empty(d.numel(), dtype=torch.int32, device=self.device)
        count = torch.empty(1, dtype=torch.int32, device=self.device)
        _lib.check(self.lib.sacenv_compact_done(d.data_ptr(), d.numel(), ids.data_ptr(),
                                                count.data_ptr(), self.stream))
        self._keep_c = d
        return ids, count

    def reset_done(self, done=None) -> torch.Tensor:
        ids, count = self.compact_done(done)
        _lib.check(self.lib.sacenv_boat_reset_list(self._pp, self._ptr, ids.data_ptr(),
                                                   count.data_ptr(), self.stream))
        self._keep = (ids, count)
        return self.obs

    def reset_explicit(self, env_ids, start_y, knots=None) -> torch.Tensor:
        ids = torch.as_tensor(env_ids, dtype=torch.int32, device=self.device).contiguous()
        sy = torch.as_tensor(start_y, dtype=torch.int32, device=self.device).contiguous()
        kn = None
        if knots is not None:
            kn = torch.as_tensor(knots, dtype=torch.float64, device=self.device).contiguous()
        _lib.check(self.lib.sacenv_boat_reset_explicit(
            self._pp, self._ptr, ids.data_ptr(), ids.numel(), sy.data_ptr(),
            None if kn is None else kn.data_ptr(), self.stream))
        self._keep = (ids, sy, kn)
        return self.obs

    def check_actions(self, actions: torch.Tensor) -> None:
        if not isinstance(actions, torch.Tensor):
            raise TypeError("actions must be a torch tensor on the env's device")
        if actions.dtype != torch.float32 or not actions.is_contiguous():
            raise ValueError("actions must be a contiguous float32 tensor")
        if actions.numel() != self.num_envs:
            raise ValueError(f"actions must hold num_envs={self.num_envs} values, got {actions.numel()}")
        if actions.device != self.device:
            raise ValueError(f"actions are on {actions.device}, the env on {self.device}")

    def step_async(self, actions: torch.Tensor) -> None:
        self.check_actions(actions)
        _lib.check(self.lib.sacenv_boat_step(self._pp, self._ptr, actions.data_ptr(), self.stream))
        self._after_step()

    def step_pooled_async(self, actions: torch.Tensor, trans_row: torch.Tensor) -> None:
        self.check_actions(actions)
        nb = _lib.trans_bytes(self.params.experiment) * self.n_pad
        if (trans_row.dtype != torch.uint8 or trans_row.device != self.device
                or trans_row.numel() != nb or not trans_row.is_contiguous()):
            raise ValueError(f"trans_row must be a contiguous uint8 device tensor of {nb} bytes")
        _lib.check(self.lib.sacenv_boat_step_pooled(self._pp, self._ptr, actions.data_ptr(),
                                                    trans_row.data_ptr(), self.stream))
        self._after_step()

    def first_obs_template(self) -> torch.Tensor:
        from .config import first_obs_template
        return torch.from_numpy(first_obs_template(self.cfg))

    def rollout(self, actions, records=None, final_obs=None):
        a = torch.as_tensor(actions, device=self.device)
        if a.dtype != torch.float32:
            a = a.to(torch.float32)
        K = int(a.shape[0])
        a = a.reshape(K, self.num_envs).contiguous()
        if self.autoreset and K > _lib.REFILL_PERIOD:
            raise ValueError(f"rollout of more than {_lib.REFILL_PERIOD} steps in autoreset mode")
        if self.autoreset and self.auto_refill and self._since_refill + K > _lib.REFILL_PERIOD:
            self.refill()
        if records is None:
            records = torch.empty((K, RECORD_BYTES * self.n_pad), dtype=torch.uint8, device=self.device)
        _lib.check(self.lib.sacenv_boat_rollout(
            self._pp, self._ptr, a.data_ptr(), K, records.data_ptr(),
            None if final_obs is None else final_obs.data_ptr(), self.stream))
        self._keep_roll = a
        if self.autoreset:
            self._since_refill += K
        return records, final_obs

    def segment_async(self, actions: torch.Tensor, n_steps: int | None = None, *, act_ready=None,
                      step_done=None, seq0: int = 0, trans=None, trans_stride: int = 0, stage=None,
                      stage_marks=None) -> None:
        K = int(actions.shape[0]) if n_steps is None else int(n_steps)
        if (not isinstance(actions, torch.Tensor) or actions.dtype != torch.float32
                or actions.device != self.device or actions.dim() != 2
                or actions.shape[1] != self.num_envs or actions.stride(1) != 1 or actions.shape[0] < K):
            raise ValueError(f"actions must be a float32 [>= {K}, {self.num_envs}] device tensor with "
                             "contiguous rows")
        if self.autoreset and K > _lib.REFILL_PERIOD:
            raise ValueError(f"a segment of more than {_lib.REFILL_PERIOD} steps in autoreset mode")
        if self.autoreset and self.auto_refill and self._since_refill + K > _lib.REFILL_PERIOD:
            self.refill()
        nw = self.n_pad // 64
        for name, f in (("act_ready", act_ready), ("step_done", step_done)):
            if f is not None and (f.dtype not in (torch.int32, torch.uint32) or f.numel() < nw
                                  or f.device != self.device or not f.is_contiguous()):
                raise ValueError(f"{name} must be a contiguous 32-bit device tensor of n_pad/64 = {nw}")
        if trans is not None:
            nb = _lib.trans_bytes(self.params.experiment) * self.n_pad
            if (trans.dtype != torch.uint8 or trans.device != self.device or not trans.is_contiguous()
                    or trans.numel() < (K - 1) * int(trans_stride) + nb):
                raise ValueError("trans must be a contiguous uint8 device tensor holding K rows")
        if stage is not None:
            if (stage.dtype != torch.uint8 or stage.device != self.device or not stage.is_contiguous()
                    or stage.numel() < K * 64 * self.n_pad):
                raise ValueError("stage must be a contiguous uint8 device tensor of n_steps x 64 x n_pad bytes")
            if stage_marks is not None and (stage_marks.dtype != torch.int64 or stage_marks.device != self.device
                                            or not stage_marks.is_contiguous()
                                            or stage_marks.numel() < self.n_pad * -(-K // 64)):
                raise ValueError("stage_marks must be a contiguous int64 device tensor of n_pad x ceil(n_steps/64)")
        _lib.check(self.lib.sacenv_boat_segment(
            self._pp, self._ptr, actions.data_ptr(), int(actions.stride(0)), K,
            None if act_ready is None else act_ready.data_ptr(),
            None if step_done is None else step_done.data_ptr(), int(seq0) & 0xFFFFFFFF,
            None if trans is None else trans.data_ptr(), int(trans_stride),
            None if stage is None else stage.data_ptr(), None if stage_marks is None else stage_marks.data_ptr(),
            self.stream))
        self._keep_seg = (actions, act_ready, step_done, trans, stage, stage_marks)
        if self.autoreset:
            self._since_refill += K

    def record_views(self, rec: torch.Tensor):
        NP, N = self.n_pad, self.num_envs
        col = lambda a, b: rec[a * NP: b * NP]
        obs = col(_lib.REC_OBS, _lib.REC_REWARD).view(torch.float32).view(NP, _lib.OBS_DIM)[:N]
        return (obs, col(_lib.REC_REWARD, _lib.REC_DONE).view(torch.float32)[:N],
                col(_lib.REC_DONE, _lib.REC_TERM)[:N], col(_lib.REC_TERM, RECORD_BYTES)[:N])

    def _after_step(self) -> None:
        if self.autoreset:
            self._since_refill += 1
            if self.auto_refill and self._since_refill >= _lib.REFILL_PERIOD:
                self.refill()

    def refill(self) -> None:
        _lib.check(self.lib.sacenv_boat_refill(self._pp, self._ptr, self.stream))
        self._since_refill = 0

    def check_status(self) -> None:
        bits = int(self.status[1].item())
        if bits & _lib.STATUS_SLOT_UNDERFLOW:
            raise _lib.SacenvError("slot underflow: more than REFILL_PERIOD steps without refill()")
        if bits & _lib.STATUS_LIST_TIMEOUT:
            raise _lib.SacenvError("refill listing timed out: a listing workgroup never published")
        if bits & _lib.STATUS_HANDOFF_TIMEOUT:
            raise _lib.SacenvError("segment hand-off timed out: an action row's flag never came; "
                                   "hand-off launches on this arena now step nothing")

    def step(self, actions):
        a = torch.as_tensor(actions, device=self.device)
        if a.dtype != torch.float32:
            a = a.to(torch.float32)
        a = a.reshape(self.num_envs).contiguous()
        self._last_action = a
        self.step_async(a)
        info = {"term": self.term, "final_obs": self.final_obs,
                "final_ep_reward": self.final_ep_reward, "counters": self.counters}
        return self.obs, self.reward, self.done, info

    def wind_eval(self, env_ids, idx):
        ids = torch.as_tensor(env_ids, dtype=torch.int32, device=self.device).contiguous()
        ix = torch.as_tensor(idx, dtype=torch.int32, device=self.device).contiguous()
        if ids.shape != ix.shape:
            raise ValueError("env_ids and idx must have the same shape")
        v = torch.empty(ids.shape, dtype=torch.float64, device=self.device)
        a = torch.empty_like(v)
        _lib.check(self.lib.sacenv_boat_wind_eval(self._pp, self._ptr, ids.data_ptr(),
                                                  ix.data_ptr(), ids.numel(), v.data_ptr(),
                                                  a.data_ptr(), self.stream))
        self._keep = (ids, ix)
        return v, a

    def state_dict(self) -> dict:
        torch.cuda.synchronize(self.device)
        d = {k: getattr(self, k).cpu().numpy() for k in
             ("s_x", "s_y", "s_r", "v_x", "v_y", "v_r", "rudder", "t", "ep_reward", "index")}
        d["start_y"] = self.start_y.cpu().numpy()
        d["fuel"] = int(self.cfg.fuel) - d["index"].astype(np.int64)
        d["a_x"], d["a_y"], d["a_r"] = self.accel.cpu().numpy()
        return d

    @property
    def counters_dict(self) -> dict:
        c = self.counters.cpu().numpy().astype(np.int64)
        return {name: c[k] for k, name in enumerate(_lib.TERM_NAMES[1:6])}
```

Baseline: 51.41 billion.

## Fuse refill pipeline into single span kernel with inline spline fit and twist

Replaces the multi-kernel refill path (need-mask scan with lookback, compacted refill list, draw kernel, separate fit kernel and MT look-ahead blocks) with one kernel, k_refill_span. Each block scans a 64-env span part directly, compacts needy lanes with ballots, prefetches the next RNG window, draws knots, fits the spline in LDS and twists the Mersenne state in place. This removes several kernel launches, the global scan and the intermediate knot round-trip through memory. In exchange every span is scanned even when few envs need a refill, per-wave work is more serialized, and the helper grid sizing changes.

```diff
diff --git a/sac-agent_amd/csrc/sacenv_boat.hip b/sac-agent_amd/csrc/sacenv_boat.hip
--- a/sac-agent_amd/csrc/sacenv_boat.hip
+++ b/sac-agent_amd/csrc/sacenv_boat.hip
@@ -48,11 +48,8 @@
     for (int j = 0; j < n; ++j) g[i * n + j] = r[i][j];
 }
 
-constexpr int kMaskThreads = 1024;
-
 __global__ void __launch_bounds__(kWave) k_seed(SacenvBoatParams p, Arena A, const uint32_t* __restrict__ seeds) {
   const int e = blockIdx.x * kWave + threadIdx.x;
-  if (e < A.nwaves()) A.refill_mask()[e] = 0ull;
   if (e >= p.n_envs) return;
   uint32_t x = seeds[e];
   uint32_t* key = A.mt_key() + (int64_t)e * kMtN;
@@ -154,236 +151,212 @@
   if (t == 0) *count = base_s;
 }
 
-#ifdef SACENV_STAMPS
-#define REFILL_STAMP(slot, ...)                                     \
-  do {                                                              \
-    asm volatile("" ::__VA_ARGS__);                                 \
-    (slot) = __builtin_amdgcn_s_memrealtime();                      \
-  } while (0)
-constexpr int kRefillStamps = 24;
-#else
-#define REFILL_STAMP(slot, ...) \
-  do {                          \
-  } while (0)
-#endif
-
 constexpr int kGroupLanes = 16;
 constexpr int kGroups = kWave / kGroupLanes;
-__global__ void __launch_bounds__(kWave) k_refill(SacenvBoatParams p, Arena A) {
-  __shared__ RngLds lds;
+constexpr int kSpanParts = 8;
+
+__device__ __forceinline__ int lanes_below(unsigned long long m) {
+  return (int)__builtin_amdgcn_mbcnt_hi((uint32_t)(m >> 32), __builtin_amdgcn_mbcnt_lo((uint32_t)m, 0u));
+}
+__device__ __forceinline__ int formed_here(int x) {
+  asm volatile("" : "+v"(x));
+  return x;
+}
+__device__ __forceinline__ void wave_mem_sync() {
+  __builtin_amdgcn_fence(__ATOMIC_RELEASE, "workgroup");
+  __builtin_amdgcn_wave_barrier();
+  __builtin_amdgcn_fence(__ATOMIC_ACQUIRE, "workgroup");
+}
+
+template <int kKnots>
+__global__ void __launch_bounds__(kWave) __attribute__((amdgpu_waves_per_eu(4)))
+k_refill_span(SacenvBoatParams p, Arena A, Tail T) {
+  __shared__ __attribute__((aligned(16))) FitLds lds;
   const int lane = threadIdx.x;
-#ifdef SACENV_STAMPS
-  uint64_t stm[kRefillStamps] = {};
-  int n_st = 0;
-#endif
-  REFILL_STAMP(stm[0], "s"(lane));
-  const int total = __builtin_amdgcn_readfirstlane(A.status()[2]);
-  REFILL_STAMP(stm[1], "s"(total));
   if (blockIdx.x == 0 && lane == 0) A.status()[0] += 1;
-  const int G = (int)gridDim.x;
   const int g = lane / kGroupLanes, gl = lane % kGroupLanes;
-  const int nk = p.n_knots;
+  constexpr bool kFull = kKnots == 8, grp_ok = kKnots <= 8;
+  const int nk = kFull ? 8 : p.n_knots;
   const int ndraw = n_curves(p.experiment);
   const int ncurves = owner_curves(p);
   const int need = 2 * nk * ndraw;
   const int nwords = kGroupLanes + need;
-  const bool grp_ok = nk <= 8;
+  const bool fits = grp_ok && ncurves > 0;
   const uint32_t rng = (uint32_t)(2 * p.start_y_half - 1), mask = range_mask32(rng);
-  const int np_ = (int)A.np;
-  int r0 = blockIdx.x * kGroups;
-  int rq = r0 + g < np_ ? r0 + g : 0;
-  int e_n = A.refill_list(0)[rq], f_n = A.refill_list(1)[rq], c_n = A.refill_list(2)[rq], p_n = A.cons_snap()[rq];
-  for (; r0 < total; r0 += kGroups * G) {
-    const int rr = r0 + g;
-    const bool ok = rr < total;
-    const int e = ok ? e_n : 0;
-    const int c = ok ? c_n : 0;
-    const int f0 = ok ? f_n : 0;
-    const int pos = ok ? (p_n & kMtPosMask) : kMtN;
-    const bool nx = ok && (p_n & kMtNextOk) != 0;
-    if (r0 + kGroups * G < total) {
-      rq = rr + kGroups * G < np_ ? rr + kGroups * G : 0;
-      e_n = A.refill_list(0)[rq], f_n = A.refill_list(1)[rq], c_n = A.refill_list(2)[rq], p_n = A.cons_snap()[rq];
-    }
-    if (ok && c >= f0 && gl == 0) atomicOr(&A.status()[1], SACENV_STATUS_SLOT_UNDERFLOW);
-    const int f_end = ok && f0 < c + kSlots ? c + kSlots : f0;
-    int f_next = f0, pos_next = pos;
-    bool live = ok && f0 < f_end && grp_ok;
-    uint32_t* const gw = lds.blk[0] + g * 3 * kGroupLanes;
+  const int cc = gl / 8, jk = gl % 8;
+  const bool knot = cc < ncurves && jk < nk;
+  const int jr = jk < nk ? jk : nk - 1;
+  IvGrid ig = interval_grid(p, jk < nk - 1 ? jk : 0);
+  ig.valid = ig.valid && fits && jk < nk - 1;
+  uint32_t* const gw = lds.blk[0] + g * 3 * kGroupLanes;
+  double* const gy = reinterpret_cast<double*>(lds.blk[1]) + g * kGroupLanes + cc * 8;
+  double* const gg = reinterpret_cast<double*>(lds.blk[1]) + kWave;
+  auto stage_g = [&] {
+    const int r = lane / 8, k = lane % 8;
+    if (fits) gg[lane] = kFull || (r < nk && k < nk) ? T.g[r * nk + k] : 0.0;
+    wave_lds_sync();
+  };
+  stage_g();
+  auto window = [&](int e, int pos, bool on, uint32_t(&w)[3]) {
+    const int64_t eo = (int64_t)e * kMtN;
+#pragma unroll
+    for (int q = 0; q < 3; ++q) {
+      const int i = pos + gl + kGroupLanes * q;
+      const uint32_t* src = i < kMtN ? A.mt_key() + eo + i : A.mt_next() + eo + (i - kMtN);
+      w[q] = on && gl + kGroupLanes * q < nwords ? *src : 0u;
+    }
+  };
+  const int items = A.nwaves() * kSpanParts;
 #pragma unroll 1
-    while (__ballot(live) != 0ull) {
-      bool fast = live && pos_next + nwords <= (nx ? 2 * kMtN : kMtN);
-      const int64_t eo = (int64_t)e * kMtN;
-      uint32_t w[3];
+  for (int item = blockIdx.x; item < items; item += (int)gridDim.x) {
+    const int span = item / kSpanParts, part = item % kSpanParts;
+    const int e0 = span * kWave, e_l = e0 + lane;
+    const bool valid = e_l < p.n_envs;
+    int c_l = 0, f_l = 0, mp_l = kMtN | kMtNextOk;
+    if (valid) {
+      c_l = A.i32(U_CONS)[e_l];
+      f_l = A.i32(U_FILL)[e_l];
+      mp_l = A.i32(U_MTPOS)[e_l];
+    }
+    const bool own = valid && lane % kSpanParts == part;
+    const bool mine = own && f_l < c_l + kSlots;
+    const int fe_l = c_l + kSlots;
+    if (mine && c_l >= f_l) atomicOr(&A.status()[1], SACENV_STATUS_SLOT_UNDERFLOW);
+    if (mine) A.i32(U_FILL)[e_l] = fe_l;
+    const unsigned long long mm = __ballot(mine);
+    const int qi = lanes_below(mm);
+    const int npass = (__popcll(mm) + kGroups - 1) / kGroups;
+    auto group_lane = [&](int t) {
+      int sl = -1;
 #pragma unroll
-      for (int q = 0; q < 3; ++q) {
-        const int i = pos_next + gl + kGroupLanes * q;
-        const uint32_t* src = i < kMtN ? A.mt_key() + eo + i : A.mt_next() + eo + (i - kMtN);
-        w[q] = fast && gl + kGroupLanes * q < nwords ? mt_temper(*src) : 0u;
+      for (int k = 0; k < kGroups; ++k) {
+        const unsigned long long b = __ballot(mine && qi == t * kGroups + k);
+        if (g == k && b != 0ull) sl = __ffsll((long long)b) - 1;
+      }
+      return sl;
+    };
+    int sl_n, f_n = 0, fe_n = 0, mp_n = 0;
+    uint32_t w_n[3];
+    auto fetch = [&](int t) {
+      sl_n = group_lane(t);
+      const int s = sl_n < 0 ? 0 : sl_n;
+      f_n = __shfl(f_l, s), fe_n = __shfl(fe_l, s), mp_n = __shfl(mp_l, s);
+      const bool on = sl_n >= 0 && grp_ok &&
+                      (mp_n & kMtPosMask) + nwords <= ((mp_n & kMtNextOk) != 0 ? 2 * kMtN : kMtN);
+      window(e0 + s, mp_n & kMtPosMask, on, w_n);
+    };
+    if (npass > 0) fetch(0);
+    bool wave_drew = false;
+#pragma unroll 1
+    for (int t = 0; t < npass; ++t) {
+      const int sl = sl_n;
+      const bool ok = sl >= 0;
+      const int e = e0 + (ok ? sl : 0);
+      const int f0 = f_n, f_end = ok ? fe_n : f_n;
+      const int pos = ok ? (mp_n & kMtPosMask) : kMtN;
+      const bool nx = ok && (mp_n & kMtNextOk) != 0;
+      uint32_t wp[3] = {w_n[0], w_n[1], w_n[2]};
+      if (t + 1 < npass) fetch(t + 1);
+      int f_next = f0, pos_next = pos;
+      bool live = ok && grp_ok;
+      bool pre = true;
+#pragma unroll 1
+      while (__ballot(live) != 0ull) {
+        bool fast = live && pos_next + nwords <= (nx ? 2 * kMtN : kMtN);
+        if (!pre) window(e, pos_next, fast, wp);
+        pre = false;
+        uint32_t w[3];
+#pragma unroll
+        for (int q = 0; q < 3; ++q) w[q] = mt_temper(wp[q]);
+        wave_lds_sync();
+#pragma unroll
+        for (int q = 0; q < 3; ++q) gw[gl + kGroupLanes * q] = w[q];
+        const unsigned long long acc = __ballot(fast && (w[0] & mask) <= rng);
+        const uint32_t gacc = (uint32_t)(acc >> (kGroupLanes * g)) & 0xFFFFu;
+        fast = fast && gacc != 0u;
+        const int k = fast ? __builtin_ctz(gacc) : 0;
+        wave_lds_sync();
+        const int slot = f_next % kSlots;
+        double yv = 0.0;
+        if (knot) {
+          const int src = k + 1 + cc * 2 * nk + 2 * jk;
+          yv = res53(gw[src], gw[src + 1]);
+          if (fast && A.rk) A.knots_raw()[A.wix(slot, cc, jk, e)] = yv;
+        }
+        if (fast && gl == 0) A.i32(U_STARTY)[(int64_t)slot * A.np + e] = -p.start_y_half + (int32_t)(gw[k] & mask);
+        if (fits) {
+          if (knot) gy[jk] = yv;
+          wave_lds_sync();
+          double mv;
+          fit_group<kFull>(p, gg + 8 * jr, ig, gy, cc, nk, yv, mv);
+          if (fast && knot)
+            *reinterpret_cast<double2*>(A.wind_knots() + 2 * A.wix(slot, cc, jk, e)) = double2{yv, mv};
+        }
+        if (fast) {
+          f_next = f_next + 1;
+          pos_next = pos_next + k + 1 + need;
+        }
+        live = fast && f_next < f_end;
+      }
+      const int mp_new = pos_next | (nx ? kMtNextOk : 0);
+#pragma unroll
+      for (int k = 0; k < kGroups; ++k) {
+        const int s = __builtin_amdgcn_readlane(sl, k * kGroupLanes);
+        const int v = __builtin_amdgcn_readlane(mp_new, k * kGroupLanes);
+        if (s >= 0 && lane == s) mp_l = v;
       }
       wave_lds_sync();
-#pragma unroll
-      for (int q = 0; q < 3; ++q) gw[gl + kGroupLanes * q] = w[q];
-      const unsigned long long acc = __ballot(fast && (w[0] & mask) <= rng);
-      const uint32_t gacc = (uint32_t)(acc >> (kGroupLanes * g)) & 0xFFFFu;
-      fast = fast && gacc != 0u;
-      const int k = fast ? __builtin_ctz(gacc) : 0;
-      wave_lds_sync();
-      REFILL_STAMP(stm[2], "v"(k));
-      if (fast) {
-        const int slot = f_next % kSlots;
-        const int cc = gl / 8, jj = gl % 8;
-        if (cc < ncurves && jj < nk) {
-          const int src = k + 1 + cc * 2 * nk + 2 * jj;
-          const double kv = res53(gw[src], gw[src + 1]);
-          A.wind_knots()[2 * A.wix(slot, cc, jj, e)] = kv;
-          if (A.rk) A.knots_raw()[A.wix(slot, cc, jj, e)] = kv;
+#pragma unroll 1
+      for (int k = 0; k < kGroups; ++k) {
+        const int src = k * kGroupLanes;
+        const int s = __builtin_amdgcn_readlane(sl, src);
+        if (s < 0) break;
+        const int fe = __builtin_amdgcn_readlane(f_end, src);
+        int f = __builtin_amdgcn_readlane(f_next, src);
+        if (f >= fe) continue;
+        int pj = __builtin_amdgcn_readlane(pos_next, src);
+        const int ej = e0 + s;
+        wave_drew = true;
+        const int ln = formed_here(lane);
+        for (; f < fe; ++f) {
+          int pj_out = 0;
+          const int32_t start_y = draw_knots_wave(p, A, lds, ej, ln, nullptr, nullptr, pj, false, 0u, &pj_out);
+          pj = pj_out;
+          __syncthreads();
+          store_draw(p, A, lds, ej, f % kSlots, start_y, ln);
+          if constexpr (!grp_ok) {
+            fit_store_wave(p, A, lds, T.g, ej, f % kSlots, ln);
+          } else if (fits) {
+            double yv = knot ? lds.y[cc][jk] : 0.0, mv;
+            wave_lds_sync();
+            stage_g();
+            if (knot) gy[jk] = yv;
+            wave_lds_sync();
+            fit_group<kFull>(p, gg + 8 * jr, ig, gy, cc, nk, yv, mv);
+            if (g == 0 && knot)
+              *reinterpret_cast<double2*>(A.wind_knots() + 2 * A.wix(f % kSlots, cc, jk, ej)) = double2{yv, mv};
+            __syncthreads();
+          }
         }
-        if (gl == 0) {
-          A.i32(U_STARTY)[(int64_t)slot * A.np + e] = -p.start_y_half + (int32_t)(gw[k] & mask);
-          A.i32(U_MTPOS)[e] = (pos_next + k + 1 + need) | (nx ? kMtNextOk : 0);
-        }
-        f_next = f_next + 1;
-        pos_next = pos_next + k + 1 + need;
+        if (lane == s) mp_l = pj;
       }
-      live = fast && f_next < f_end;
-    }
+    }
+    if (wave_drew) wave_mem_sync();
+    const int ix = mp_l & kMtPosMask;
+    const bool adv_l = (mp_l & kMtNextOk) != 0 && ix > kMtN;
+    const bool tw = own && grp_ok && ((mp_l & kMtNextOk) == 0 || ix > kMtN);
+    unsigned long long tm = __ballot(tw);
+#pragma unroll 1
+    while (tm != 0ull) {
+      const int j = __ffsll((long long)tm) - 1;
+      tm &= tm - 1ull;
+      const bool adv = __builtin_amdgcn_readlane((int)adv_l, j) != 0;
+      uint32_t* const key = A.mt_key() + (int64_t)(e0 + j) * kMtN;
+      uint32_t* const nxt = A.mt_next() + (int64_t)(e0 + j) * kMtN;
+      mt_twist_regs(adv ? nxt : key, nxt, adv ? key : nullptr, formed_here(lane));
+    }
+    if (mine || tw) A.i32(U_MTPOS)[e_l] = tw ? ((ix - (adv_l ? kMtN : 0)) | kMtNextOk) : mp_l;
     wave_lds_sync();
-#pragma unroll 1
-    for (int j = 0; j < kGroups; ++j) {
-      const int src = j * kGroupLanes;
-      if (__builtin_amdgcn_readlane((int)ok, src) == 0) break;
-      const int ej = __builtin_amdgcn_readlane(e, src);
-      const int fe = __builtin_amdgcn_readlane(f_end, src);
-      int f = __builtin_amdgcn_readlane(f_next, src);
-      const int pj = __builtin_amdgcn_readlane(pos_next, src);
-      bool first = true;
-      for (; f < fe; ++f) {
-        const int32_t start_y = draw_knots_wave(p, A, lds, ej, lane, nullptr, nullptr, first ? pj : -1);
-#ifdef SACENV_STAMPS
-        const int sb = 3 + (n_st < 18 ? n_st : 18);
-        ++n_st;
-#endif
-        REFILL_STAMP(stm[sb], "v"(start_y));
-        first = false;
-        __syncthreads();
-        store_draw(p, A, lds, ej, f % kSlots, start_y, lane, true);
-        __syncthreads();
-      }
-      if (lane == 0) {
-        A.i32(U_FILL)[ej] = fe;
-        A.refill_list(1)[r0 + j] = __builtin_amdgcn_readlane(f0, src);
-        A.refill_list(2)[r0 + j] = fe;
-      }
-    }
-  }
-#ifdef SACENV_STAMPS
-  stm[22] = __builtin_amdgcn_s_memrealtime();
-  stm[23] = (uint64_t)n_st;
-  if (lane == 0 && (int64_t)(blockIdx.x + 1) * kRefillStamps * 8 <= 24 * A.np) {
-    uint64_t* d = reinterpret_cast<uint64_t*>(A.accel()) + (int64_t)blockIdx.x * kRefillStamps;
-    for (int i = 0; i < kRefillStamps; ++i) d[i] = stm[i];
-  }
-#endif
-}
-
-template <int GS, bool kFull>
-__global__ void __launch_bounds__(kWave) k_refill_fit(SacenvBoatParams p, Arena A, Tail T) {
-  const int lane = threadIdx.x;
-  const int ahead = (int)(A.np / kAheadEnvs);
-  if ((int)blockIdx.x < ahead) {
-    mt_ahead(p, A, (int)blockIdx.x, lane);
-    return;
-  }
-  const int fb = (int)blockIdx.x - ahead, fgrid = (int)gridDim.x - ahead;
-  const int nc = p.use_wind_table ? 0 : n_curves(p.experiment);
-  const int nk = kFull ? GS : p.n_knots;
-  const int items = A.status()[2] * nc;
-#ifdef SACENV_STAMPS
-  const uint64_t st0 = __builtin_amdgcn_s_memrealtime();
-  uint64_t* const fst = reinterpret_cast<uint64_t*>(A.reward64()) + 2 * (int64_t)blockIdx.x;
-  const bool fst_ok = lane == 0 && (int64_t)(blockIdx.x + 1) * 16 <= 8 * A.np;
-  if (fst_ok) fst[0] = st0, fst[1] = 0;
-#endif
-  if (items == 0 || fb * (kWave / GS) >= items) return;
-  const int j = lane & (GS - 1);
-  const int jj = j < nk ? j : nk - 1, j1 = jj + 1 < nk ? jj + 1 : jj;
-  double gr[GS];
-#pragma unroll
-  for (int k = 0; k < GS; ++k) gr[k] = kFull || k < nk ? T.g[jj * nk + k] : 0.0;
-  IvGrid ig = interval_grid(p, j < nk - 1 ? j : 0);
-  ig.valid = ig.valid && j < nk - 1;
-  const int per = kWave / GS;
-  for (int base = fb * per; base < items; base += fgrid * per) {
-    const int item = base + lane / GS;
-    if (item >= items) break;
-    fit_group<GS, kFull>(p, A, gr, ig, item, j, jj, j1, nc);
-  }
-#ifdef SACENV_STAMPS
-  __syncthreads();
-  if (fst_ok) fst[1] = __builtin_amdgcn_s_memrealtime();
-#endif
-}
-
-__device__ __forceinline__ unsigned long long lookback_load(const unsigned long long* w) {
-  return __hip_atomic_load(w, __ATOMIC_RELAXED, __HIP_MEMORY_SCOPE_AGENT);
-}
-__global__ void __launch_bounds__(kMaskThreads) k_need_masks(SacenvBoatParams p, Arena A) {
-  __shared__ int wcnt[kMaskThreads / kWave];
-  const int t = threadIdx.x, lane = t & (kWave - 1), wv = t >> 6;
-  const int nw = A.nwaves(), b = (int)blockIdx.x;
-  const int w = b * (kMaskThreads / kWave) + wv, e = w * kWave + lane;
-  const uint32_t epoch = (uint32_t)A.status()[0] + 1u;
-  bool need = false;
-  int c = 0, fl = 0, mp = 0;
-  if (w < nw && e < p.n_envs) {
-    c = A.i32(U_CONS)[e];
-    fl = A.i32(U_FILL)[e];
-    mp = A.i32(U_MTPOS)[e];
-    need = fl < c + kSlots;
-  }
-  const unsigned long long m = __ballot(need);
-  if (lane == 0) wcnt[wv] = __popcll(m);
-  __syncthreads();
-  if (t < kWave) {
-    unsigned long long* const look = A.refill_mask();
-    const int cnt = t < kMaskThreads / kWave ? wcnt[t] : 0;
-    const int incl = wave_incl_scan(cnt);
-    const int total = __builtin_amdgcn_readlane(incl, kMaskThreads / kWave - 1);
-    if (t == 0)
-      __hip_atomic_store(look + b, ((unsigned long long)epoch << 32) | (uint32_t)total, __ATOMIC_RELAXED,
-                         __HIP_MEMORY_SCOPE_AGENT);
-    int before = 0;
-    for (int q0 = 0; q0 < b; q0 += kWave) {
-      const int q = q0 + t;
-      unsigned long long x = q < b ? lookback_load(look + q) : ((unsigned long long)epoch << 32);
-      for (uint32_t it = 0; __ballot((uint32_t)(x >> 32) != epoch) != 0ull; ++it) {
-        if (it >= kSpinLimit) {
-          if (t == 0) atomicOr(&A.status()[1], SACENV_STATUS_LIST_TIMEOUT);
-          break;
-        }
-        __builtin_amdgcn_s_sleep(1);
-        if ((uint32_t)(x >> 32) != epoch) x = lookback_load(look + q);
-      }
-      int v = (uint32_t)(x >> 32) == epoch ? (int)(uint32_t)x : 0;
-      v += __shfl_xor(v, 32);
-      v += __shfl_xor(v, 16);
-      v += __shfl_xor(v, 8);
-      v += __shfl_xor(v, 4);
-      v += __shfl_xor(v, 2);
-      v += __shfl_xor(v, 1);
-      before += v;
-    }
-    if (t < kMaskThreads / kWave) wcnt[t] = before + incl - cnt;
-    if (t == 0 && b == (int)gridDim.x - 1) A.status()[2] = before + total;
-  }
-  __syncthreads();
-  if (need) {
-    const int r = wcnt[wv] + __popcll(m & ((1ull << lane) - 1ull));
-    A.refill_list(0)[r] = e;
-    A.refill_list(1)[r] = fl;
-    A.refill_list(2)[r] = c;
-    A.cons_snap()[r] = mp;
   }
 }
 
@@ -535,7 +508,6 @@
 using StepKernel = void (*)(SacenvBoatParams, Arena, Tail, const float*, int, MixedToys, char*);
 using RolloutKernel = void (*)(SacenvBoatParams, Arena, Tail, const float*, int, RollArgs);
 using MixedRolloutKernel = void (*)(SacenvBoatParams, Arena, Tail, const float*, int, RollArgs, int, MixedToys);
-using FitKernel = void (*)(SacenvBoatParams, Arena, Tail);
 
 template <int kNc, bool kTIdx>
 struct Owner {
@@ -600,13 +572,6 @@
     using O = decltype(o);
     return lean ? k_rollout_mixed<O::nc, O::ti, true> : k_rollout_mixed<O::nc, O::ti>;
   });
-}
-
-FitKernel refill_fit_kernel(int n_knots) {
-  return n_knots == 8   ? k_refill_fit<8, true>
-         : n_knots < 8  ? k_refill_fit<8, false>
-         : n_knots == 16 ? k_refill_fit<16, true>
-                         : k_refill_fit<16, false>;
 }
 
 RollArgs arena_roll_args(const Arena& A) {
@@ -874,14 +839,10 @@
   if (arena == nullptr) return SACENV_E_NULL;
   if (!p->autoreset) return SACENV_E_MODE;
   const Arena A = make_arena(*p, arena);
-  const unsigned mask_blocks = (unsigned)((A.np / kWave + kMaskThreads / kWave - 1) / (kMaskThreads / kWave));
-  hipLaunchKernelGGL(k_need_masks, dim3(mask_blocks), dim3(kMaskThreads), 0, (hipStream_t)stream, *p, A);
-  if ((rc = launch_status())) return rc;
-  hipLaunchKernelGGL(k_refill, dim3(p->n_helpers), dim3(kWave), 0, (hipStream_t)stream, *p, A);
-  if ((rc = launch_status())) return rc;
-  const int fit_blocks = 8192 + (int)(A.np / kAheadEnvs);
-  hipLaunchKernelGGL(refill_fit_kernel(p->n_knots), dim3(fit_blocks), dim3(kWave), 0, (hipStream_t)stream, *p, A,
-                     make_tail(*p, arena));
+  hipLaunchKernelGGL(p->n_knots == 8  ? k_refill_span<8>
+                     : p->n_knots < 8 ? k_refill_span<0>
+                                      : k_refill_span<16>, dim3(p->n_helpers), dim3(kWave), 0,
+                     (hipStream_t)stream, *p, A, make_tail(*p, arena));
   return launch_status();
 }
 
diff --git a/sac-agent_amd/csrc/sacenv_boat_arena.h b/sac-agent_amd/csrc/sacenv_boat_arena.h
--- a/sac-agent_amd/csrc/sacenv_boat_arena.h
+++ b/sac-agent_amd/csrc/sacenv_boat_arena.h
@@ -125,15 +125,9 @@
   __device__ __forceinline__ double* accel() const { return at<double>(ur() + R_AX); }
   __device__ __forceinline__ double* reward64() const { return at<double>(ur() + R_REWARD64); }
   __device__ __forceinline__ char* tail() const { return b + off_refill_mask(ur(), np); }
-  __device__ __forceinline__ unsigned long long* refill_mask() const {
-    return reinterpret_cast<unsigned long long*>(tail());
-  }
-
-  __device__ __forceinline__ int32_t* cons_snap() const { return i32(U_CSNAP); }
   __device__ __forceinline__ int32_t* status() const {
     return reinterpret_cast<int32_t*>(tail() + refill_mask_bytes(np));
   }
-  __device__ __forceinline__ int32_t* refill_list(int k) const { return i32(U_LIST + 4 * k); }
   __device__ __forceinline__ int64_t wix(int slot, int c, int k, int e) const {
     return (((int64_t)e * kSlots + slot) * 2 + c) * nk + k;
   }
diff --git a/sac-agent_amd/csrc/sacenv_boat_draw.h b/sac-agent_amd/csrc/sacenv_boat_draw.h
--- a/sac-agent_amd/csrc/sacenv_boat_draw.h
+++ b/sac-agent_amd/csrc/sacenv_boat_draw.h
@@ -18,8 +18,10 @@
   uint32_t blk[2][kMtN];
   double y[2][kMaxK];
 };
-struct DrawLds : RngLds {
+struct FitLds : RngLds {
   double m[2][kMaxK];
+};
+struct DrawLds : FitLds {
   double g[kMaxK * kMaxK];
 };
 
@@ -32,7 +34,8 @@
 
 __device__ int32_t draw_knots_wave(const SacenvBoatParams& p, const Arena& A, RngLds& l, int e,
                                    int lane, const int32_t* ex_start_y, const double* ex_knots,
-                                   int pos0 = -1, bool have_w0 = false, uint32_t w0_pre = 0u) {
+                                   int pos0 = -1, bool have_w0 = false, uint32_t w0_pre = 0u,
+                                   int* pos_out = nullptr) {
   const int nk = p.n_knots;
   const int ndraw = n_curves(p.experiment);
   const int ncurves = owner_curves(p);
@@ -91,11 +94,12 @@
     }
   }
   mt_finish(st, l, A.i32(U_MTPOS) + e, lane);
+  if (pos_out != nullptr) *pos_out = st.pos;
   return -p.start_y_half + (int32_t)val;
 }
 
-__device__ void fit_store_wave(const SacenvBoatParams& p, const Arena& A, DrawLds& l, int e, int slot,
-                               int lane) {
+__device__ void fit_store_wave(const SacenvBoatParams& p, const Arena& A, FitLds& l, const double* g, int e,
+                               int slot, int lane) {
   const int nk = p.n_knots;
   const int ncurves = owner_curves(p);
   if (ncurves == 0) return;
@@ -107,7 +111,7 @@
     yv = l.y[c][j];
 #pragma unroll
     for (int k = 0; k < kMaxK; ++k)
-      if (k < nk) mv += l.g[j * nk + k] * l.y[c][k];
+      if (k < nk) mv += g[j * nk + k] * l.y[c][k];
     l.m[c][j] = mv;
   }
   __syncthreads();
@@ -139,13 +143,12 @@
 }
 
 __device__ __forceinline__ void store_draw(const SacenvBoatParams& p, const Arena& A, const RngLds& l,
-                                           int e, int slot, int32_t start_y, int lane, bool raw = false) {
+                                           int e, int slot, int32_t start_y, int lane) {
   const int nk = p.n_knots;
   const int ncurves = owner_curves(p);
   if (lane == 0) A.i32(U_STARTY)[(int64_t)slot * A.np + e] = start_y;
   const int c = lane >> 4, j = lane & 15;
   if (c < ncurves && j < nk) {
-    if (raw) A.wind_knots()[2 * A.wix(slot, c, j, e)] = l.y[c][j];
     if (A.rk) A.knots_raw()[A.wix(slot, c, j, e)] = l.y[c][j];
   }
 }
@@ -156,7 +159,7 @@
   const int32_t start_y = draw_knots_wave(p, A, l, e, lane, ex_start_y, ex_knots);
   __syncthreads();
   store_draw(p, A, l, e, slot, start_y, lane);
-  fit_store_wave(p, A, l, e, slot, lane);
+  fit_store_wave(p, A, l, l.g, e, slot, lane);
   return start_y;
 }
 
@@ -188,7 +191,6 @@
   return make_obs(p, obs_const(T), 0.0, 0.0, 0.0, s_y, 0.0, 0.0, 0.0, 0.0, 0.0, 0.0, (double)p.fuel0);
 }
 
-constexpr int kAheadEnvs = 8;
 __device__ __forceinline__ void mt_twist_regs(const uint32_t* o, uint32_t* n, uint32_t* cur, int lane) {
   constexpr int kD = kMtN - kMtM;
   uint32_t a0[4], a1[4], a2[4], b0[4], b1[4], c0[4], c1[4];
@@ -232,27 +234,4 @@
   }
 }
 
-__device__ __forceinline__ void mt_ahead(const SacenvBoatParams& p, const Arena& A, int b, int lane) {
-  const int e0 = b * kAheadEnvs;
-  int v = 0;
-  bool need = false;
-  if (lane < kAheadEnvs && e0 + lane < p.n_envs && p.n_knots <= 8) {
-    v = A.i32(U_MTPOS)[e0 + lane];
-    need = (v & kMtNextOk) == 0 || (v & kMtPosMask) > kMtN;
-  }
-  unsigned long long m = __ballot(need);
-#pragma unroll 1
-  while (m != 0ull) {
-    const int j = __ffsll((long long)m) - 1;
-    m &= m - 1ull;
-    const int e = e0 + j;
-    const int vj = __builtin_amdgcn_readlane(v, j);
-    const bool adv = (vj & kMtNextOk) != 0 && (vj & kMtPosMask) > kMtN;
-    uint32_t* const key = A.mt_key() + (int64_t)e * kMtN;
-    uint32_t* const nxt = A.mt_next() + (int64_t)e * kMtN;
-    mt_twist_regs(adv ? nxt : key, nxt, adv ? key : nullptr, lane);
-    if (lane == 0) A.i32(U_MTPOS)[e] = ((vj & kMtPosMask) - (adv ? kMtN : 0)) | kMtNextOk;
-  }
-}
-
-}
+}
diff --git a/sac-agent_amd/csrc/sacenv_boat_wind.h b/sac-agent_amd/csrc/sacenv_boat_wind.h
--- a/sac-agent_amd/csrc/sacenv_boat_wind.h
+++ b/sac-agent_amd/csrc/sacenv_boat_wind.h
@@ -211,36 +211,25 @@
   }
 }
 
-template <int GS, bool kFull>
-__device__ __forceinline__ void fit_group(const SacenvBoatParams& p, const Arena& A, const double (&gr)[GS],
-                                          const IvGrid& ig, int item, int j, int jj, int j1, int nc) {
-  const int nk = kFull ? GS : p.n_knots;
-  const int rr = item / nc, c = item - rr * nc;
-  const int e = A.refill_list(0)[rr], f0 = A.refill_list(1)[rr], f1 = A.refill_list(2)[rr];
-  for (int f = f0; f < f1; ++f) {
-    const int slot = f % kSlots;
-    const double* kr = A.wind_knots() + 2 * A.wix(slot, c, 0, e);
-    double yk[GS];
+template <bool kFull>
+__device__ __forceinline__ void fit_group(const SacenvBoatParams& p, const double* grow, const IvGrid& ig,
+                                          const double* gy, int c, int nk, double& yv, double& mv) {
+  double yk[8];
 #pragma unroll
-    for (int k = 0; k < GS; ++k) yk[k] = kr[2 * (kFull || k < nk ? k : nk - 1)];
-    double yv = kr[2 * jj];
-    const double y1 = kr[2 * j1];
-    double mv = 0.0;
+  for (int k = 0; k < 8; ++k) yk[k] = gy[kFull || k < nk ? k : nk - 1];
+  const double y1 = next_lane_f64(yv);
+  mv = 0.0;
 #pragma unroll
-    for (int k = 0; k < GS; ++k) {
-      const double s = mv + gr[k] * yk[k];
-      mv = kFull || k < nk ? s : mv;
-    }
-    const double m1 = next_lane_f64(mv);
-    double mn, mx;
-    interval_extrema_on<1>(p, ig, 0, yv, y1, mv, m1, mn, mx);
-    mn = group_min<GS>(mn);
-    mx = group_max<GS>(mx);
-    if (kFull || j < nk) {
-      fold_knot(p, c, mn, mx, yv, mv);
-      *reinterpret_cast<double2*>(A.wind_knots() + 2 * A.wix(slot, c, j, e)) = double2{yv, mv};
-    }
-  }
-}
-
-}
+  for (int k = 0; k < 8; ++k) {
+    const double s = mv + grow[k] * yk[k];
+    mv = kFull || k < nk ? s : mv;
+  }
+  const double m1 = next_lane_f64(mv);
+  double mn, mx;
+  interval_extrema_on<1>(p, ig, 0, yv, y1, mv, m1, mn, mx);
+  mn = group_min<8>(mn);
+  mx = group_max<8>(mx);
+  fold_knot(p, c, mn, mx, yv, mv);
+}
+
+}
diff --git a/sac-agent_amd/sacenv/vec_env.py b/sac-agent_amd/sacenv/vec_env.py
--- a/sac-agent_amd/sacenv/vec_env.py
+++ b/sac-agent_amd/sacenv/vec_env.py
@@ -30,7 +30,7 @@
         self.auto_refill = bool(auto_refill)
         self._since_refill = 0
         if n_helpers is None:
-            n_helpers = max(1024, ((N + 63) // 64 * 64) * 3 // 16)
+            n_helpers = max(1024, (N + 63) // 64 * 8)
         flags = ((_lib.OUT_KNOTS if record_knots else 0) | (_lib.OUT_ACCEL if record_accel else 0)
                  | (_lib.OUT_REWARD64 if record_reward64 else 0))
         self.params = make_params(self.cfg, N, max_episode_steps=max_episode_steps,
```

Measured after the change: 51.64 billion (median of 3 runs). No clear change (+0.4%).
